# LBM-EPFL/MaD

Hardware: NVIDIA B200
Metric: voxels/sec scale-space+detect+describe(+match) (higher is better)
Workload: dtype f32 grids, f64 line accumulation, u8 x u8 -> s32 matching

## Files before the change

### include/mad_b200.h

```cpp
#ifndef MAD_B200_H
#define MAD_B200_H

#include <stddef.h>
#include <stdint.h>

#ifdef __cplusplus
extern "C" {
#endif

#define MAD_OK 0
#define MAD_ERR_ARG (-1)
#define MAD_ERR_CUDA (-2)
#define MAD_ERR_CAPACITY (-3)
#define MAD_ERR_NODEVICE (-4)

#define MAD_MAX_ORI 36
#define MAD_DSC_LEN 1024
#define MAD_DSC_REFUSED (1 << 30)

typedef struct MadKeypoint {
    int32_t vox[3];
    int32_t oct;
    float off[3];
    float val;
    int32_t peak[3];
    int32_t accepted;
} MadKeypoint;

typedef struct MadOriented {
    int32_t kp;
    int16_t main_bin;
    int16_t sec_bin;
} MadOriented;

typedef struct MadZoneTable {
    int32_t n_zones;
    int32_t n_belts;
    const double* bounds;
    const int32_t* belt_first;
    const double* belt_phi;
    const void* fast;
} MadZoneTable;

#define MAD_ZONE_FAST_BYTES 2048
int mad_zone_fast_build(const MadZoneTable* zones_host, void* fast_out, void* stream);

const char* mad_last_error_string(void);
int mad_version(void);
int mad_device_info(int* sm_count, int* cc_major, int* cc_minor);

int mad_publish_small(const void* src_dev, void* dst_host_mapped, int bytes, void* stream);

int mad_copy_to_host(const void* src_dev, void* dst_host_mapped, long long bytes, int n_ctas, void* stream);

long long mad_launch_count(void);
int mad_profile_enable(int on);
int mad_profile_count(void);
int mad_profile_get(int i, const char** name, float* ms);
int mad_profile_reset(void);

int mad_grid_max(const float* grid, long long n, float* out_max_ord, void* stream);
float mad_grid_max_decode(unsigned int ord);
int mad_threshold_normalise(float* grid, long long n, float isovalue, float vmax, int divide, void* stream);
int mad_grid_bbox(const float* grid, int nx, int ny, int nz, int* bbox6, void* stream);
int mad_crop_pad3d(const float* in, int nx, int ny, int nz, int x0, int y0, int z0, int cx, int cy, int cz,
                   int pad, float* out, void* stream);

int mad_pad3d(const float* in, int nx, int ny, int nz, int pad, float* out, void* stream);

size_t mad_upsample_workspace_bytes(int bx, int by, int bz);
int mad_upsample_presmooth(const float* base, int bx, int by, int bz,
                           const double* gauss_w_host, int radius,
                           float* up, void* workspace, size_t workspace_bytes, void* stream);

size_t mad_log_gauss_workspace_bytes(int nx, int ny, int nz);
int mad_log_gauss(const float* grid, int nx, int ny, int nz,
                  const double* w0_host, const double* w2_host, int radius, float scale,
                  float* log_out, float* gauss_out, void* workspace, size_t workspace_bytes,
                  int exact_f64, void* stream);

int mad_gradient(const float* gauss, int nx, int ny, int nz, float* grad4, void* stream);
size_t mad_gradient_tiles(int nx, int ny, int nz);
int mad_gradient_mark(const MadKeypoint* kp, int n_kp, const int* dims_oct_host, int reach_oct0, int reach_oct1,
                      uint8_t* flags_oct0, uint8_t* flags_oct1, void* stream);
int mad_gradient_masked(const float* gauss, int nx, int ny, int nz, float* grad4, uint8_t* flags, void* stream);

int mad_detect(const float* log_grid, int nx, int ny, int nz, int oct, int border,
               float threshold, MadKeypoint* cand, int cap, int* count, void* stream);

size_t mad_sort_keypoints_workspace_bytes(int n);
int mad_sort_keypoints(const MadKeypoint* cand, int n, const int* dims_oct_host,
                       MadKeypoint* out, int* out_count,
                       void* workspace, size_t workspace_bytes, void* stream);

int mad_orient(const float* grad4_oct0, const float* grad4_oct1, const int* dims_oct_host,
               const MadKeypoint* kp, int n_kp, int r, const MadZoneTable* zones112_host,
               const double* r1_table, int lim_main, int lim_sec,
               int32_t* n_ori, int32_t* slots, void* stream);

size_t mad_compact_oriented_workspace_bytes(int n_kp);
int mad_compact_oriented(const int32_t* n_ori, const int32_t* slots, int n_kp,
                         MadOriented* oriented, int cap, int* out_count,
                         void* workspace, size_t workspace_bytes, void* stream);

int mad_describe(const float* grad4_oct0, const float* grad4_oct1, const int* dims_oct_host,
                 const MadKeypoint* kp, const MadOriented* oriented, int n_oriented, int r,
                 const MadZoneTable* zones16_host, const double* rf_table, const double* rf_inv_table,
                 int rf_zones, int16_t* dsc, void* stream);

typedef struct MadDscSet {
    const int16_t* dsc;
    const void* half;
    const int32_t* norm2;
    const uint8_t* u8;
    const float* rnorm;
    int32_t rows;
    int32_t rows_padded;
    int32_t max_entry;
    int32_t max_norm2;
} MadDscSet;

int mad_dsc_prepare(const int16_t* dsc, int rows, int rows_padded, int32_t* norm2, float* rnorm,
                    uint8_t* u8, int32_t* max_entry, int32_t* max_norm2, void* stream);
int mad_dsc_norms(const int16_t* dsc, int rows, int32_t* norm2, void* stream);
int mad_dsc_to_half(const int16_t* dsc, int rows, int rows_padded, void* half_out, void* stream);

int mad_match_segments(int M, int N, int impl);
int mad_match_count(const MadDscSet* hi, const MadDscSet* lo, double cc, int n_seg, int32_t* seg_count, int impl,
                    void* stream);
int mad_match_fill(const MadDscSet* hi, const MadDscSet* lo, double cc, int n_seg, const int64_t* seg_offset,
                   int32_t* pair_hi, int32_t* pair_lo, double* pair_score, int impl, void* stream);
size_t mad_exclusive_scan_workspace_bytes(int n);
int mad_exclusive_scan_i32_to_i64(const int32_t* in, int n, int64_t* out, int64_t* total,
                                  void* workspace, size_t workspace_bytes, void* stream);

int mad_match_pairs(const MadDscSet* hi, const MadDscSet* lo, double cc, uint64_t* cand_key, int32_t* cand_dot,
                    uint64_t cap, uint64_t* count, void* stream);
size_t mad_match_pairs_finish_workspace_bytes(long long n);
int mad_match_pairs_finish(const uint64_t* cand_key, const int32_t* cand_dot, long long n, int hi_rows, int lo_rows,
                           const int32_t* hi_n2, const int32_t* lo_n2, int32_t* pair_hi, int32_t* pair_lo,
                           double* pair_score, void* workspace, size_t workspace_bytes, void* stream);
int mad_match_pairs_finish_dot(const uint64_t* cand_key, const int32_t* cand_dot, long long n, int hi_rows, int lo_rows,
                               int32_t* pair_hi, int32_t* pair_lo, int32_t* pair_dot, void* workspace, size_t workspace_bytes,
                               void* stream);

size_t mad_match_topk_workspace_bytes(int M, int N, int k, int impl);
int mad_match_topk(const MadDscSet* hi, const MadDscSet* lo, int k, int lo_index_base,
                   int32_t* topk_idx, double* topk_score, void* workspace, size_t workspace_bytes,
                   int impl, void* stream);
#define MAD_TOPK_INCOMPLETE (-2)
int mad_topk_merge(const int32_t* idx_in, const double* score_in, int G, int M, int k,
                   int32_t* idx_out, double* score_out, void* stream);

int mad_mark_used(const int32_t* idx, long long n, uint8_t* used, void* stream);
int mad_repeatability(const int32_t* pair_hi, const int32_t* pair_lo, const double* pair_score, long long n_pairs,
                      const double* hi_subv, const double* lo_subv, const int32_t* hi_meta, const int32_t* lo_meta,
                      const double* rf_table, const double* rf_inv_table, int rf_zones,
                      const double* hi_cloud, int n_hi_cloud, const double* lo_sorted, const int32_t* cell_start,
                      const uint32_t* near_bits, const double* grid_org_host, const int* grid_dims_host,
                      double dist, double* results, void* stream);
int mad_repeat_counts(const int32_t* pair_hi, const int32_t* pair_lo, long long p0, long long p1,
                      const double* hi_subv, const double* lo_subv, const int32_t* hi_meta, const int32_t* lo_meta,
                      const double* rf_table, const double* rf_inv_table, int rf_zones,
                      const double* hi_cloud, int n_hi_cloud, const double* lo_sorted, const int32_t* cell_start,
                      const uint32_t* near_bits, const double* grid_org_host, const int* grid_dims_host,
                      double dist, int32_t* counts, void* stream);
int mad_repeat_rows(const int32_t* pair_hi, const int32_t* pair_lo, const double* pair_score, long long n_pairs,
                    const double* hi_subv, const double* lo_subv, const int32_t* hi_meta, const int32_t* lo_meta,
                    const double* rf_table, const double* rf_inv_table, int rf_zones, const int32_t* counts,
                    int n_hi_cloud, double* results, void* stream);

size_t mad_anchor_cloud_workspace_bytes(int n_rows);
int mad_anchor_cloud(const double* subv, const uint8_t* used, int n_rows, double cell, double* cloud, double* grid_org,
                     long long* info, void* workspace, size_t workspace_bytes, void* stream);
size_t mad_cloud_grid_workspace_bytes(int n);
int mad_cloud_grid(const double* cloud, int n, const double* grid_org, const long long* grid_dims_host, double cell,
                   double* sorted, int32_t* cell_start, uint32_t* near_bits, void* workspace, size_t workspace_bytes,
                   void* stream);

int mad_density_splat(const double* xyz, const double* mass, int n_atoms, const double* min_host, double voxelsp,
                      int margin, int px, int py, int pz, double* grid, void* stream);
int mad_normalise_f64(double* grid, long long n, void* scratch8, void* stream);
int mad_conv_full_f64(const double* in, long long outer, int n, long long inner, const double* w_dev, int radius,
                      void* out, int out_is_f32, void* stream);

size_t mad_box_scores_workspace_bytes(int ex, int ey, int ez);
int mad_box_scores(const float* g1, int nx1, int ny1, int nz1, const float* g2, int nx2, int ny2, int nz2,
                   const int* box_host, float isovalue, double* out8, void* workspace, size_t workspace_bytes,
                   void* stream);
int mad_grid_count_gt(const float* grid, long long n, float thr, unsigned long long* out, void* stream);
int mad_mask_with(float* g1, int nx1, int ny1, int nz1, const float* g2, int nx2, int ny2, int nz2,
                  const int* shift_host, const int* lo_host, const int* hi_host, void* stream);
int mad_refine_rigid(const float* grad4, int nx, int ny, int nz, const double* px, const double* py, const double* pz,
                     double voxsp, const double* init, const double* center, const double* max_dist, int n_problems,
                     int n_atoms, int n_steps, double max_step, double min_step, double* coords_out, double* meta_out,
                     void* stream);

#ifdef __cplusplus
}
#endif
#endif
```

### mad_b200/_lib.py

```python
import ctypes as C
import os

import numpy as np

HERE = os.path.dirname(os.path.abspath(__file__))
LIB_PATH = os.path.join(HERE, "libmad_b200.so")


class MadError(RuntimeError):
    pass


if not os.path.exists(LIB_PATH):
    raise ImportError(
        "mad_b200: %s is missing -- build the CUDA library first (python -m mad_b200.build). "
        "There is no CPU fallback." % LIB_PATH)

lib = C.CDLL(LIB_PATH)

KEYPOINT_DTYPE = np.dtype([("vox", "<i4", 3), ("oct", "<i4"), ("off", "<f4", 3), ("val", "<f4"),
                           ("peak", "<i4", 3), ("accepted", "<i4")])
ORIENTED_DTYPE = np.dtype([("kp", "<i4"), ("main", "<i2"), ("sec", "<i2")])
assert KEYPOINT_DTYPE.itemsize == 48 and ORIENTED_DTYPE.itemsize == 8
MAX_ORI = 36
DSC_LEN = 1024
DSC_REFUSED = 1 << 30
TOPK_INCOMPLETE = -2
TOPK_MAX = 32
ZONE_FAST_BYTES = 2048


class MadZoneTable(C.Structure):
    _fields_ = [("n_zones", C.c_int32), ("n_belts", C.c_int32), ("bounds", C.c_void_p),
                ("belt_first", C.c_void_p), ("belt_phi", C.c_void_p), ("fast", C.c_void_p)]


class MadDscSet(C.Structure):
    _fields_ = [("dsc", C.c_void_p), ("half", C.c_void_p), ("norm2", C.c_void_p), ("u8", C.c_void_p),
                ("rnorm", C.c_void_p), ("rows", C.c_int32), ("rows_padded", C.c_int32), ("max_entry", C.c_int32),
                ("max_norm2", C.c_int32)]


_P = C.c_void_p
_I = C.c_int
_SZ = C.c_size_t

SIGNATURES = {
    "mad_last_error_string": (C.c_char_p, []),
    "mad_version": (_I, []),
    "mad_device_info": (_I, [C.POINTER(_I), C.POINTER(_I), C.POINTER(_I)]),
    "mad_launch_count": (C.c_longlong, []),
    "mad_profile_enable": (_I, [_I]),
    "mad_profile_count": (_I, []),
    "mad_profile_get": (_I, [_I, C.POINTER(C.c_char_p), C.POINTER(C.c_float)]),
    "mad_profile_reset": (_I, []),
    "mad_publish_small": (_I, [_P, _P, _I, _P]),
    "mad_copy_to_host": (_I, [_P, _P, C.c_longlong, _I, _P]),
    "mad_zone_fast_build": (_I, [C.POINTER(MadZoneTable), _P, _P]),
    "mad_grid_max": (_I, [_P, C.c_longlong, _P, _P]),
    "mad_grid_max_decode": (C.c_float, [C.c_uint]),
    "mad_threshold_normalise": (_I, [_P, C.c_longlong, C.c_float, C.c_float, _I, _P]),
    "mad_grid_bbox": (_I, [_P, _I, _I, _I, _P, _P]),
    "mad_crop_pad3d": (_I, [_P, _I, _I, _I, _I, _I, _I, _I, _I, _I, _I, _P, _P]),
    "mad_pad3d": (_I, [_P, _I, _I, _I, _I, _P, _P]),
    "mad_upsample_workspace_bytes": (_SZ, [_I, _I, _I]),
    "mad_upsample_presmooth": (_I, [_P, _I, _I, _I, _P, _I, _P, _P, _SZ, _P]),
    "mad_log_gauss_workspace_bytes": (_SZ, [_I, _I, _I]),
    "mad_log_gauss": (_I, [_P, _I, _I, _I, _P, _P, _I, C.c_float, _P, _P, _P, _SZ, _I, _P]),
    "mad_gradient": (_I, [_P, _I, _I, _I, _P, _P]),
    "mad_gradient_tiles": (_SZ, [_I, _I, _I]),
    "mad_gradient_mark": (_I, [_P, _I, _P, _I, _I, _P, _P, _P]),
    "mad_gradient_masked": (_I, [_P, _I, _I, _I, _P, _P, _P]),
    "mad_detect": (_I, [_P, _I, _I, _I, _I, _I, C.c_float, _P, _I, _P, _P]),
    "mad_sort_keypoints_workspace_bytes": (_SZ, [_I]),
    "mad_sort_keypoints": (_I, [_P, _I, _P, _P, _P, _P, _SZ, _P]),
    "mad_orient": (_I, [_P, _P, _P, _P, _I, _I, C.POINTER(MadZoneTable), _P, _I, _I, _P, _P, _P]),
    "mad_compact_oriented_workspace_bytes": (_SZ, [_I]),
    "mad_compact_oriented": (_I, [_P, _P, _I, _P, _I, _P, _P, _SZ, _P]),
    "mad_describe": (_I, [_P, _P, _P, _P, _P, _I, _I, C.POINTER(MadZoneTable), _P, _P, _I, _P, _P]),
    "mad_dsc_prepare": (_I, [_P, _I, _I, _P, _P, _P, _P, _P, _P]),
    "mad_match_pairs": (_I, [C.POINTER(MadDscSet), C.POINTER(MadDscSet), C.c_double, _P, _P, C.c_uint64, _P, _P]),
    "mad_match_pairs_finish_workspace_bytes": (_SZ, [C.c_longlong]),
    "mad_match_pairs_finish": (_I, [_P, _P, C.c_longlong, _I, _I, _P, _P, _P, _P, _P, _P, _SZ, _P]),
    "mad_match_pairs_finish_dot": (_I, [_P, _P, C.c_longlong, _I, _I, _P, _P, _P, _P, _SZ, _P]),
    "mad_dsc_norms": (_I, [_P, _I, _P, _P]),
    "mad_dsc_to_half": (_I, [_P, _I, _I, _P, _P]),
    "mad_match_segments": (_I, [_I, _I, _I]),
    "mad_match_count": (_I, [C.POINTER(MadDscSet), C.POINTER(MadDscSet), C.c_double, _I, _P, _I, _P]),
    "mad_match_fill": (_I, [C.POINTER(MadDscSet), C.POINTER(MadDscSet), C.c_double, _I, _P, _P, _P, _P, _I, _P]),
    "mad_exclusive_scan_workspace_bytes": (_SZ, [_I]),
    "mad_exclusive_scan_i32_to_i64": (_I, [_P, _I, _P, _P, _P, _SZ, _P]),
    "mad_match_topk_workspace_bytes": (_SZ, [_I, _I, _I, _I]),
    "mad_match_topk": (_I, [C.POINTER(MadDscSet), C.POINTER(MadDscSet), _I, _I, _P, _P, _P, _SZ, _I, _P]),
    "mad_topk_merge": (_I, [_P, _P, _I, _I, _I, _P, _P, _P]),
    "mad_density_splat": (_I, [_P, _P, _I, _P, C.c_double, _I, _I, _I, _I, _P, _P]),
    "mad_normalise_f64": (_I, [_P, C.c_longlong, _P, _P]),
    "mad_conv_full_f64": (_I, [_P, C.c_longlong, _I, C.c_longlong, _P, _I, _P, _I, _P]),
    "mad_mark_used": (_I, [_P, C.c_longlong, _P, _P]),
    "mad_repeatability": (_I, [_P, _P, _P, C.c_longlong, _P, _P, _P, _P, _P, _P, _I, _P, _I, _P, _P, _P, _P, _P,
                               C.c_double, _P, _P]),
    "mad_repeat_counts": (_I, [_P, _P, C.c_longlong, C.c_longlong, _P, _P, _P, _P, _P, _P, _I, _P, _I, _P, _P, _P, _P, _P,
                               C.c_double, _P, _P]),
    "mad_repeat_rows": (_I, [_P, _P, _P, C.c_longlong, _P, _P, _P, _P, _P, _P, _I, _P, _I, _P, _P]),
    "mad_anchor_cloud_workspace_bytes": (_SZ, [_I]),
    "mad_anchor_cloud": (_I, [_P, _P, _I, C.c_double, _P, _P, _P, _P, _SZ, _P]),
    "mad_cloud_grid_workspace_bytes": (_SZ, [_I]),
    "mad_cloud_grid": (_I, [_P, _I, _P, _P, C.c_double, _P, _P, _P, _P, _SZ, _P]),
    "mad_box_scores_workspace_bytes": (_SZ, [_I, _I, _I]),
    "mad_box_scores": (_I, [_P, _I, _I, _I, _P, _I, _I, _I, _P, C.c_float, _P, _P, _SZ, _P]),
    "mad_grid_count_gt": (_I, [_P, C.c_longlong, C.c_float, _P, _P]),
    "mad_mask_with": (_I, [_P, _I, _I, _I, _P, _I, _I, _I, _P, _P, _P, _P]),
    "mad_refine_rigid": (_I, [_P, _I, _I, _I, _P, _P, _P, C.c_double, _P, _P, _P, _I, _I, _I, C.c_double, C.c_double,
                              _P, _P, _P]),
}

for _name, (_res, _args) in SIGNATURES.items():
    _f = getattr(lib, _name)
    _f.restype = _res
    _f.argtypes = _args


def last_error():
    s = lib.mad_last_error_string()
    return s.decode() if s else ""


def check(rc, what):
    if rc != 0:
        raise MadError("%s failed with status %d: %s" % (what, rc, last_error()))


def call(name, *args):
    check(getattr(lib, name)(*args), name)
```

### mad_b200/csrc/match_common.cuh

```cuda
#pragma once
#include <math.h>
#include "common.cuh"

#define MAD_TOPK_MAX 32

__host__ __device__ __forceinline__ double mad_score(int dot, double n2a, double n2b) {
    const double p = n2a * n2b;
    return p > 0.0 ? (double)dot / sqrt(p) : 0.0;
}

__host__ __device__ __forceinline__ void mad_topk_insert(double* bs, int* bi, int k, double s, int id) {
    const double ls = bs[k - 1];
    const int li = bi[k - 1];
    if (!(s > ls || (s == ls && (li < 0 || id < li)))) return;
    int q = k - 1;
    while (q > 0) {
        const double ps = bs[q - 1];
        const int pi = bi[q - 1];
        if (s > ps || (s == ps && (pi < 0 || id < pi))) { bs[q] = ps; bi[q] = pi; --q; }
        else break;
    }
    bs[q] = s;
    bi[q] = id;
}

__host__ __device__ __forceinline__ bool mad_topk_before(double s, int id, double ps, int pi) {
    return s > ps || (s == ps && (pi < 0 || id < pi));
}

__device__ __forceinline__ void mad_top8_insert(double (&bs)[8], int (&bi)[8], double s, int id) {
    bool c[8];
#pragma unroll
    for (int q = 0; q < 8; ++q) c[q] = mad_topk_before(s, id, bs[q], bi[q]);
#pragma unroll
    for (int q = 7; q >= 1; --q) {
        bs[q] = c[q - 1] ? bs[q - 1] : (c[q] ? s : bs[q]);
        bi[q] = c[q - 1] ? bi[q - 1] : (c[q] ? id : bi[q]);
    }
    bs[0] = c[0] ? s : bs[0];
    bi[0] = c[0] ? id : bi[0];
}

static __device__ __noinline__ bool mad_score_before_nl(int d, int n, int id, int pd, int pn, int pi, double n2a) {
    return mad_topk_before(mad_score(d, n2a, (double)n), id, mad_score(pd, n2a, (double)pn), pi);
}
__device__ __forceinline__ bool mad_score32_before(float s, int d, int n, int id, float ps, int pd, int pn, int pi, double n2a) {
    if (pi < 0) return true;
    const float tol = 4e-6f * fmaxf(s, ps);
    if (s > ps + tol) return true;
    if (s < ps - tol) return false;
    return mad_score_before_nl(d, n, id, pd, pn, pi, n2a);
}

__device__ __forceinline__ void mad_top8f_insert(float (&ts)[8], int (&td)[8], int (&tn)[8], int (&bi)[8], bool active, float s,
                                                 int d, int n, int id, double n2a) {
    bool c[8];
    bool amb = false;
#pragma unroll
    for (int q = 0; q < 8; ++q) {
        const float ps = ts[q];
        const bool empty = bi[q] < 0;
        const float tol = 4e-6f * fmaxf(s, ps);
        const bool gt = s > ps + tol, lt = s < ps - tol;
        c[q] = active && (empty || gt);
        amb |= active && !empty && !gt && !lt;
    }
    if (__any_sync(0xFFFFFFFFu, amb)) {
#pragma unroll
        for (int q = 0; q < 8; ++q) c[q] = active && mad_score32_before(s, d, n, id, ts[q], td[q], tn[q], bi[q], n2a);
    }
#pragma unroll
    for (int q = 7; q >= 1; --q) {
        ts[q] = c[q - 1] ? ts[q - 1] : (c[q] ? s : ts[q]);
        td[q] = c[q - 1] ? td[q - 1] : (c[q] ? d : td[q]);
        tn[q] = c[q - 1] ? tn[q - 1] : (c[q] ? n : tn[q]);
        bi[q] = c[q - 1] ? bi[q - 1] : (c[q] ? id : bi[q]);
    }
    ts[0] = c[0] ? s : ts[0];
    td[0] = c[0] ? d : td[0];
    tn[0] = c[0] ? n : tn[0];
    bi[0] = c[0] ? id : bi[0];
}

__device__ __forceinline__ void mad_st_release_cta(volatile int* p, int v) {
    asm volatile("st.release.cta.shared::cta.s32 [%0], %1;" ::"r"((uint32_t)__cvta_generic_to_shared((const void*)p)), "r"(v) : "memory");
}
__device__ __forceinline__ int mad_ld_acquire_cta(volatile int* p) {
    int v;
    asm volatile("ld.acquire.cta.shared::cta.s32 %0, [%1];" : "=r"(v) : "r"((uint32_t)__cvta_generic_to_shared((const void*)p)) : "memory");
    return v;
}

__device__ __forceinline__ uint32_t mad_select32(const uint32_t (&v)[32], int j) {
    uint32_t a[16];
#pragma unroll
    for (int i = 0; i < 16; ++i) a[i] = (j & 1) ? v[2 * i + 1] : v[2 * i];
    uint32_t b[8];
#pragma unroll
    for (int i = 0; i < 8; ++i) b[i] = (j & 2) ? a[2 * i + 1] : a[2 * i];
    uint32_t c[4];
#pragma unroll
    for (int i = 0; i < 4; ++i) c[i] = (j & 4) ? b[2 * i + 1] : b[2 * i];
    const uint32_t d0 = (j & 8) ? c[1] : c[0], d1 = (j & 8) ? c[3] : c[2];
    return (j & 16) ? d1 : d0;
}

#define MAD_MATCH_SEG_TILE 256

int mad_check_descriptor_sets(const MadDscSet* hi, const MadDscSet* lo, const char* who);

int mad_match_simt(const int16_t* hi, int M, const int16_t* lo, int N, const int32_t* hi_n2, const int32_t* lo_n2,
                   double cc, int mode, int S, int32_t* seg_count, const int64_t* seg_offset, int32_t* pair_hi,
                   int32_t* pair_lo, double* pair_score, int k, int lo_index_base, int32_t* topk_idx,
                   double* topk_score, cudaStream_t st);

int mad_match_tc_segments(int M, int N);
int mad_match_tc(const void* hi_half, int M, int M_pad, const void* lo_half, int N, int N_pad,
                 const int32_t* hi_n2, const int32_t* lo_n2, double cc, int mode, int S, int32_t* seg_count,
                 const int64_t* seg_offset, int32_t* pair_hi, int32_t* pair_lo, double* pair_score, int k,
                 int lo_index_base, int32_t* topk_idx, double* topk_score, cudaStream_t st);
int mad_topk_merge_launch(const int32_t* idx_in, const double* score_in, int G, int M, int k, int32_t* idx_out,
                          double* score_out, cudaStream_t st);

int mad_match_u8_segments(int M, int N);
int mad_match_u8_segments_topk(int M, int N);
int mad_match_u8_pairs(const void* hi_u8, int M, int M_pad, const void* lo_u8, int N, int N_pad, const int32_t* hi_n2,
                       const int32_t* lo_n2, const float* lo_rnorm, double cc, unsigned long long* cand_key,
                       int32_t* cand_dot, unsigned long long cap, unsigned long long* count, cudaStream_t st);
int mad_match_u8_topk(const void* hi_u8, int M, int M_pad, const void* lo_u8, int N, int N_pad, const int32_t* hi_n2,
                      const int32_t* lo_n2, const float* lo_rnorm, int S, int k, int lo_index_base, int32_t* topk_idx,
                      double* topk_score, cudaStream_t st);
```

### mad_b200/csrc/match_prep.cu

```cuda
#include <cub/cub.cuh>

#include "common.cuh"
#include "match_common.cuh"

namespace {

__global__ void __launch_bounds__(256)
dsc_prepare_kernel(const int16_t* __restrict__ dsc, int rows, int rows_padded, int32_t* __restrict__ norm2,
                   float* __restrict__ rnorm, uint8_t* __restrict__ u8, int32_t* __restrict__ max_entry,
                   int32_t* __restrict__ max_norm2) {
    const int row = (int)((blockIdx.x * (long long)blockDim.x + threadIdx.x) >> 5);
    const int lane = threadIdx.x & 31;
    if (row >= rows_padded) return;
    long long acc = 0;
    int mx = 0;
    uint32_t packed[8];
    if (row < rows) {
        const uint4* src = reinterpret_cast<const uint4*>(dsc + (long long)row * MAD_DSC_LEN + lane * 32);
#pragma unroll
        for (int q = 0; q < 4; ++q) {
            const uint4 v = __ldg(src + q);
            const uint32_t w[4] = {v.x, v.y, v.z, v.w};
#pragma unroll
            for (int h = 0; h < 4; ++h) {
                const int e0 = (int)(int16_t)(w[h] & 0xFFFFu), e1 = (int)(int16_t)(w[h] >> 16);
                acc += (long long)e0 * e0 + (long long)e1 * e1;
                mx = max(mx, max(e0, e1));
                if (e0 < 0 || e1 < 0) mx = MAD_DSC_REFUSED;
                const uint32_t b0 = (uint32_t)min(max(e0, 0), 255), b1 = (uint32_t)min(max(e1, 0), 255);
                const int slot = q * 8 + h * 2;
                if ((slot & 3) == 0) packed[slot >> 2] = b0 | (b1 << 8);
                else packed[slot >> 2] |= (b0 << 16) | (b1 << 24);
            }
        }
    } else {
#pragma unroll
        for (int q = 0; q < 8; ++q) packed[q] = 0;
    }
    if (u8) {
        uint4* dst = reinterpret_cast<uint4*>(u8 + (long long)row * MAD_DSC_LEN + lane * 32);
        dst[0] = make_uint4(packed[0], packed[1], packed[2], packed[3]);
        dst[1] = make_uint4(packed[4], packed[5], packed[6], packed[7]);
    }
#pragma unroll
    for (int o = 16; o > 0; o >>= 1) {
        acc += __shfl_xor_sync(0xFFFFFFFFu, acc, o);
        mx = max(mx, __shfl_xor_sync(0xFFFFFFFFu, mx, o));
    }
    if (lane == 0) {
        if (acc > 0x7FFFFFFFLL) mx = MAD_DSC_REFUSED;
        if (row < rows) norm2[row] = (int32_t)acc;
        rnorm[row] = acc > 0 ? (float)(1.0 / sqrt((double)acc)) : 0.f;
        if (mx > 0) atomicMax(max_entry, mx);
        if (max_norm2 && acc > 0) atomicMax(max_norm2, (int32_t)min(acc, 0x7FFFFFFFLL));
    }
}

__global__ void pairs_finish_kernel(const unsigned long long* __restrict__ key, const int32_t* __restrict__ dot,
                                    long long n, unsigned long long lo_rows, const int32_t* __restrict__ hi_n2,
                                    const int32_t* __restrict__ lo_n2,
                                    int32_t* __restrict__ pair_hi, int32_t* __restrict__ pair_lo,
                                    double* __restrict__ score) {
    const long long i = blockIdx.x * (long long)blockDim.x + threadIdx.x;
    if (i >= n) return;
    const unsigned long long k = key[i];
    const int row = (int)(k / lo_rows), col = (int)(k % lo_rows);
    pair_hi[i] = row;
    pair_lo[i] = col;
    score[i] = mad_score(dot[i], (double)__ldg(hi_n2 + row), (double)__ldg(lo_n2 + col));
}

__global__ void pairs_finish_dot_kernel(const unsigned long long* __restrict__ key, const int32_t* __restrict__ dot, long long n,
                                        unsigned long long lo_rows, int32_t* __restrict__ pair_hi, int32_t* __restrict__ pair_lo,
                                        int32_t* __restrict__ pair_dot) {
    const long long i = blockIdx.x * (long long)blockDim.x + threadIdx.x;
    if (i >= n) return;
    const unsigned long long k = key[i];
    pair_hi[i] = (int)(k / lo_rows);
    pair_lo[i] = (int)(k % lo_rows);
    pair_dot[i] = dot[i];
}

__global__ void zero_u64_kernel(unsigned long long* p) { *p = 0ull; }

struct FinishLayout {
    size_t key_off, dot_off, cub_off, cub_bytes, total;
};

FinishLayout finish_layout(long long n) {
    FinishLayout L;
    const size_t nn = (size_t)(n > 0 ? n : 1);
    L.key_off = 0;
    L.dot_off = mad_align_up(nn * sizeof(unsigned long long), 256);
    L.cub_off = L.dot_off + mad_align_up(nn * sizeof(int32_t), 256);
    size_t b = 0;
    cub::DeviceRadixSort::SortPairs(nullptr, b, (const unsigned long long*)nullptr, (unsigned long long*)nullptr,
                                    (const int32_t*)nullptr, (int32_t*)nullptr, (int)nn, 0, 64);
    L.cub_bytes = mad_align_up(b, 256);
    L.total = L.cub_off + L.cub_bytes;
    return L;
}

}

extern "C" int mad_dsc_prepare(const int16_t* dsc, int rows, int rows_padded, int32_t* norm2, float* rnorm,
                               uint8_t* u8, int32_t* max_entry, int32_t* max_norm2, void* stream) {
    MAD_CHECK_ARG(rows >= 0 && rows_padded >= rows);
    if (rows_padded == 0) return MAD_OK;
    MAD_CHECK_ARG((rows == 0 || dsc) && norm2 && rnorm && max_entry);
    MAD_CHECK_ARG((reinterpret_cast<uintptr_t>(dsc) & 15) == 0 && (reinterpret_cast<uintptr_t>(u8) & 15) == 0);
    MAD_PROF("dsc_prepare_kernel", stream);
    dsc_prepare_kernel<<<(unsigned)mad_ceil_div((long long)rows_padded * 32, 256), 256, 0, (cudaStream_t)stream>>>(
        dsc, rows, rows_padded, norm2, rnorm, u8, max_entry, max_norm2);
    MAD_LAUNCH_OK();
    return MAD_OK;
}

extern "C" int mad_match_pairs(const MadDscSet* hi, const MadDscSet* lo, double cc, uint64_t* cand_key, int32_t* cand_dot,
                               uint64_t cap, uint64_t* count, void* stream) {
    MAD_CHECK_ARG(hi && lo && count && hi->rows >= 0 && lo->rows >= 0);
    cudaStream_t st = (cudaStream_t)stream;
    {
        MAD_PROF("zero_u64_kernel", st);
        zero_u64_kernel<<<1, 1, 0, st>>>(reinterpret_cast<unsigned long long*>(count));
        MAD_LAUNCH_OK();
    }
    if (hi->rows == 0 || lo->rows == 0) return MAD_OK;
    MAD_CHECK_ARG(hi->u8 && lo->u8 && hi->norm2 && lo->norm2 && lo->rnorm && cand_key && cand_dot);
    MAD_CHECK_ARG(hi->rows_padded >= hi->rows && hi->rows_padded % 128 == 0);
    MAD_CHECK_ARG(lo->rows_padded >= lo->rows && lo->rows_padded % 128 == 0);
    int rc = mad_check_descriptor_sets(hi, lo, "mad_match_pairs");
    if (rc != MAD_OK) return rc;
    if (hi->max_entry > 255 || lo->max_entry > 255) {
        mad_set_error("mad_match_pairs: descriptor entries up to %d do not fit the uint8 tensor-core operand "
                      "(use mad_match_count/mad_match_fill with impl = 2 or 1)",
                      hi->max_entry > lo->max_entry ? hi->max_entry : lo->max_entry);
        return MAD_ERR_ARG;
    }
    return mad_match_u8_pairs(hi->u8, hi->rows, hi->rows_padded, lo->u8, lo->rows, lo->rows_padded, hi->norm2, lo->norm2,
                              lo->rnorm, cc, reinterpret_cast<unsigned long long*>(cand_key), cand_dot,
                              (unsigned long long)cap, reinterpret_cast<unsigned long long*>(count), st);
}

extern "C" size_t mad_match_pairs_finish_workspace_bytes(long long n) { return finish_layout(n).total; }

static int pairs_finish_impl(const uint64_t* cand_key, const int32_t* cand_dot, long long n, int hi_rows, int lo_rows,
                             const int32_t* hi_n2, const int32_t* lo_n2, int32_t* pair_hi, int32_t* pair_lo, double* pair_score,
                             int32_t* pair_dot, void* workspace, size_t workspace_bytes, void* stream);

extern "C" int mad_match_pairs_finish(const uint64_t* cand_key, const int32_t* cand_dot, long long n, int hi_rows,
                                      int lo_rows, const int32_t* hi_n2, const int32_t* lo_n2, int32_t* pair_hi, int32_t* pair_lo,
                                      double* pair_score, void* workspace, size_t workspace_bytes, void* stream) {
    MAD_CHECK_ARG(n >= 0 && n < (1LL << 31));
    if (n == 0) return MAD_OK;
    MAD_CHECK_ARG(hi_n2 && lo_n2 && pair_score);
    return pairs_finish_impl(cand_key, cand_dot, n, hi_rows, lo_rows, hi_n2, lo_n2, pair_hi, pair_lo, pair_score, nullptr, workspace,
                             workspace_bytes, stream);
}

extern "C" int mad_match_pairs_finish_dot(const uint64_t* cand_key, const int32_t* cand_dot, long long n, int hi_rows, int lo_rows,
                                          int32_t* pair_hi, int32_t* pair_lo, int32_t* pair_dot, void* workspace,
                                          size_t workspace_bytes, void* stream) {
    MAD_CHECK_ARG(n >= 0 && n < (1LL << 31));
    if (n == 0) return MAD_OK;
    MAD_CHECK_ARG(pair_dot);
    return pairs_finish_impl(cand_key, cand_dot, n, hi_rows, lo_rows, nullptr, nullptr, pair_hi, pair_lo, nullptr, pair_dot, workspace,
                             workspace_bytes, stream);
}

static int pairs_finish_impl(const uint64_t* cand_key, const int32_t* cand_dot, long long n, int hi_rows, int lo_rows,
                             const int32_t* hi_n2, const int32_t* lo_n2, int32_t* pair_hi, int32_t* pair_lo, double* pair_score,
                             int32_t* pair_dot, void* workspace, size_t workspace_bytes, void* stream) {
    MAD_CHECK_ARG(cand_key && cand_dot && pair_hi && pair_lo && workspace && hi_rows > 0 && lo_rows > 0);
    const FinishLayout L = finish_layout(n);
    MAD_CHECK_ARG(workspace_bytes >= L.total);
    cudaStream_t st = (cudaStream_t)stream;
    char* ws = reinterpret_cast<char*>(workspace);
    unsigned long long* key_sorted = reinterpret_cast<unsigned long long*>(ws + L.key_off);
    int32_t* dot_sorted = reinterpret_cast<int32_t*>(ws + L.dot_off);
    int key_bits = 1;
    while (key_bits < 64 && (1ULL << key_bits) < (unsigned long long)hi_rows * (unsigned long long)lo_rows) ++key_bits;
    size_t b = L.cub_bytes;
    {
        MAD_PROF("cub_radix_sort_pairs", st);
        MAD_CUDA(cub::DeviceRadixSort::SortPairs(ws + L.cub_off, b, reinterpret_cast<const unsigned long long*>(cand_key),
                                                 key_sorted, cand_dot, dot_sorted, (int)n, 0, key_bits, st));
    }
    MAD_PROF("pairs_finish_kernel", st);
    if (pair_dot)
        pairs_finish_dot_kernel<<<(unsigned)mad_ceil_div(n, 256), 256, 0, st>>>(key_sorted, dot_sorted, n, (unsigned long long)lo_rows, pair_hi,
                                                                               pair_lo, pair_dot);
    else
        pairs_finish_kernel<<<(unsigned)mad_ceil_div(n, 256), 256, 0, st>>>(key_sorted, dot_sorted, n, (unsigned long long)lo_rows, hi_n2, lo_n2,
                                                                           pair_hi, pair_lo, pair_score);
    MAD_LAUNCH_OK();
    return MAD_OK;
}
```

### mad_b200/csrc/match_u8.cu

```cuda
#include <cuda.h>
#include <stdlib.h>

#include <type_traits>

#include "common.cuh"
#include "match_common.cuh"

namespace {

constexpr int BM = 128;
constexpr int BN = 128;
constexpr int BKB = 128;
constexpr int UKB = 32;
constexpr int KBLOCKS = MAD_DSC_LEN / BKB;
constexpr int STAGES = 5;
constexpr int STAGES2 = 10;
constexpr int ACCS = 4;
constexpr uint32_t KB_BYTES = BM * BKB;
constexpr uint32_t A_BYTES = KBLOCKS * KB_BYTES;
constexpr int EPI_WARPS = 8;
constexpr int THREADS = 128 + 32 * EPI_WARPS + 64;
constexpr uint32_t TMEM_COLS = 512;
constexpr unsigned long long MAD_MATCH_TIMEOUT_COUNT = 1ull << 62;
constexpr int STG = 96;
constexpr size_t STG_BYTES = (size_t)EPI_WARPS * STG * (sizeof(unsigned long long) + sizeof(int));
constexpr size_t RB_BYTES = (size_t)2 * 2 * 256 * sizeof(float);
constexpr size_t THR_BYTES = 512;
constexpr int TOP_SLOTS = 2;
constexpr int TOP_LOCAL_TILES = 4;
constexpr unsigned long long TOP_INVALID = ~0ull;
static_assert((size_t)EPI_WARPS * 2 * 32 * TOP_SLOTS * sizeof(unsigned long long) <= STG_BYTES, "TOP8 slots fit the staging area");
constexpr size_t SMEM_BYTES = 1024 + A_BYTES + (size_t)STAGES * KB_BYTES + STG_BYTES + RB_BYTES + 512 + THR_BYTES;
static_assert(SMEM_BYTES <= 232448, "shared memory budget of one sm_100 CTA");

__device__ __forceinline__ uint32_t smem_u32(const void* p) { return (uint32_t)__cvta_generic_to_shared(p); }
__device__ __forceinline__ void mbar_init(uint32_t bar, uint32_t count) {
    asm volatile("mbarrier.init.shared::cta.b64 [%0], %1;" ::"r"(bar), "r"(count) : "memory");
}
__device__ __forceinline__ void mbar_expect_tx(uint32_t bar, uint32_t bytes) {
    asm volatile("mbarrier.arrive.expect_tx.shared::cta.b64 _, [%0], %1;" ::"r"(bar), "r"(bytes) : "memory");
}
__device__ __forceinline__ void mbar_arrive(uint32_t bar) {
    asm volatile("mbarrier.arrive.shared::cta.b64 _, [%0];" ::"r"(bar) : "memory");
}
__device__ __forceinline__ void mbar_wait(uint32_t bar, uint32_t parity) {
    uint32_t done;
    do {
        asm volatile(
            "{\n\t.reg .pred p;\n\t"
            "mbarrier.try_wait.parity.shared::cta.b64 p, [%1], %2;\n\t"
            "selp.u32 %0, 1, 0, p;\n\t}"
            : "=r"(done)
            : "r"(bar), "r"(parity)
            : "memory");
    } while (!done);
}
__device__ __forceinline__ void tma_load_2d(uint32_t dst, const CUtensorMap* map, uint32_t bar, int c0, int c1) {
    asm volatile(
        "cp.async.bulk.tensor.2d.shared::cluster.global.mbarrier::complete_tx::bytes [%0], [%1, {%3, %4}], [%2];"
        ::"r"(dst), "l"(reinterpret_cast<uint64_t>(map)), "r"(bar), "r"(c0), "r"(c1)
        : "memory");
}
constexpr uint32_t kPeerBitMask = 0xFEFFFFFFu;
__device__ __forceinline__ uint32_t cluster_ctarank() {
    uint32_t r;
    asm volatile("mov.u32 %0, %%cluster_ctarank;" : "=r"(r));
    return r;
}
__device__ __forceinline__ void cluster_sync_all() {
    asm volatile("barrier.cluster.arrive.release.aligned;" ::: "memory");
    asm volatile("barrier.cluster.wait.acquire.aligned;" ::: "memory");
}
__device__ __forceinline__ void tma_load_2d_2sm(uint32_t dst, const CUtensorMap* map, uint32_t bar, int c0, int c1) {
    asm volatile(
        "cp.async.bulk.tensor.2d.cta_group::2.shared::cluster.global.mbarrier::complete_tx::bytes [%0], [%1, {%3, %4}], [%2];"
        ::"r"(dst), "l"(reinterpret_cast<uint64_t>(map)), "r"(bar & kPeerBitMask), "r"(c0), "r"(c1)
        : "memory");
}
__device__ __forceinline__ void mbar_arrive_leader(uint32_t bar) {
    asm volatile("mbarrier.arrive.shared::cluster.b64 _, [%0];" ::"r"(bar & kPeerBitMask) : "memory");
}
__device__ __forceinline__ void umma_commit_pair(uint32_t bar) {
    asm volatile("tcgen05.commit.cta_group::2.mbarrier::arrive::one.shared::cluster.multicast::cluster.b64 [%0], %1;"
                 ::"r"(bar), "h"((uint16_t)3) : "memory");
}
__device__ __forceinline__ void umma_i8_pair(uint32_t d_tmem, uint64_t a_desc, uint64_t b_desc, uint32_t idesc, uint32_t accumulate) {
    asm volatile(
        "{\n\t.reg .pred p;\n\t"
        "setp.ne.b32 p, %4, 0;\n\t"
        "tcgen05.mma.cta_group::2.kind::i8 [%0], %1, %2, %3, p;\n\t}"
        ::"r"(d_tmem), "l"(a_desc), "l"(b_desc), "r"(idesc), "r"(accumulate)
        : "memory");
}
__device__ __forceinline__ void umma_commit(uint32_t bar) {
    asm volatile("tcgen05.commit.cta_group::1.mbarrier::arrive::one.shared::cluster.b64 [%0];" ::"r"(bar) : "memory");
}
__device__ __forceinline__ void umma_i8(uint32_t d_tmem, uint64_t a_desc, uint64_t b_desc, uint32_t idesc, uint32_t accumulate) {
    asm volatile(
        "{\n\t.reg .pred p;\n\t"
        "setp.ne.b32 p, %4, 0;\n\t"
        "tcgen05.mma.cta_group::1.kind::i8 [%0], %1, %2, %3, p;\n\t}"
        ::"r"(d_tmem), "l"(a_desc), "l"(b_desc), "r"(idesc), "r"(accumulate)
        : "memory");
}
__device__ __forceinline__ void tmem_ld32(uint32_t taddr, uint32_t (&v)[32]) {
    asm volatile(
        "tcgen05.ld.sync.aligned.32x32b.x32.b32 "
        "{%0, %1, %2, %3, %4, %5, %6, %7, %8, %9, %10, %11, %12, %13, %14, %15, "
        "%16, %17, %18, %19, %20, %21, %22, %23, %24, %25, %26, %27, %28, %29, %30, %31}, [%32];"
        : "=r"(v[0]), "=r"(v[1]), "=r"(v[2]), "=r"(v[3]), "=r"(v[4]), "=r"(v[5]), "=r"(v[6]), "=r"(v[7]),
          "=r"(v[8]), "=r"(v[9]), "=r"(v[10]), "=r"(v[11]), "=r"(v[12]), "=r"(v[13]), "=r"(v[14]), "=r"(v[15]),
          "=r"(v[16]), "=r"(v[17]), "=r"(v[18]), "=r"(v[19]), "=r"(v[20]), "=r"(v[21]), "=r"(v[22]), "=r"(v[23]),
          "=r"(v[24]), "=r"(v[25]), "=r"(v[26]), "=r"(v[27]), "=r"(v[28]), "=r"(v[29]), "=r"(v[30]), "=r"(v[31])
        : "r"(taddr)
        : "memory");
}
__device__ __forceinline__ uint32_t tmem_ld1(uint32_t taddr) {
    uint32_t x;
    asm volatile("tcgen05.ld.sync.aligned.32x32b.x1.b32 {%0}, [%1];" : "=r"(x) : "r"(taddr) : "memory");
    return x;
}
__device__ __forceinline__ void tmem_ld_wait() { asm volatile("tcgen05.wait::ld.sync.aligned;" ::: "memory"); }
__device__ __forceinline__ void tc_fence_before() { asm volatile("tcgen05.fence::before_thread_sync;" ::: "memory"); }
__device__ __forceinline__ void tc_fence_after() { asm volatile("tcgen05.fence::after_thread_sync;" ::: "memory"); }

__device__ __forceinline__ uint64_t umma_smem_desc(uint32_t saddr) {
    uint64_t d = 0;
    d |= (uint64_t)((saddr & 0x3FFFFu) >> 4);
    d |= (uint64_t)1 << 16;
    d |= (uint64_t)(1024u >> 4) << 32;
    d |= (uint64_t)1 << 46;
    d |= (uint64_t)2 << 61;
    return d;
}
constexpr uint32_t kIdesc = (2u << 4) | ((uint32_t)(BN >> 3) << 17) | ((uint32_t)(BM >> 4) << 24);
constexpr uint32_t kIdescPair = (2u << 4) | ((uint32_t)((2 * BN) >> 3) << 17) | ((uint32_t)((2 * BM) >> 4) << 24);

struct U8Args {
    int M, N, S;
    int tiles_per_seg;
    const int32_t* hi_n2;
    const int32_t* lo_n2;
    const float* lo_rnorm;
    double cc;
    unsigned long long* cand_key;
    int32_t* cand_dot;
    unsigned long long cap;
    unsigned long long* count;
    int k, lo_index_base;
    int local_tiles;
    int dbg;
    int32_t* topk_idx;
    double* topk_score;
};

__device__ unsigned long long g_top_dbg[8];

enum { MODE_PAIRS = 0, MODE_TOPK = 1, MODE_TOP8 = 2 };

template <int MODE, int NCTA>
__global__ void __launch_bounds__(THREADS, 1)
match_u8_kernel(const __grid_constant__ CUtensorMap map_hi, const __grid_constant__ CUtensorMap map_lo, U8Args a) {
    constexpr int TN = (NCTA == 2) ? 2 * BN : BN;
    constexpr int NACC = (int)TMEM_COLS / TN;
    constexpr int NSTAGE = STAGES;
    constexpr uint32_t SB = KB_BYTES;
    extern __shared__ uint8_t smem_raw[];
    const uint32_t raw = smem_u32(smem_raw);
    const uint32_t base = (raw + 1023u) & ~1023u;
    uint8_t* gen = smem_raw + (base - raw);
    const uint32_t b_ring = base + A_BYTES;
    constexpr uint32_t STG_OFF = A_BYTES + STAGES * KB_BYTES;
    unsigned long long* stg_key = reinterpret_cast<unsigned long long*>(gen + STG_OFF);
    int* stg_dot = reinterpret_cast<int*>(gen + STG_OFF + EPI_WARPS * STG * sizeof(unsigned long long));
    float* s_rb = reinterpret_cast<float*>(gen + STG_OFF + (uint32_t)STG_BYTES);
    constexpr uint32_t BAR_OFF = STG_OFF + (uint32_t)(STG_BYTES + RB_BYTES);
    const uint32_t bars = base + BAR_OFF;
    auto full_bar = [&](int s) { return bars + 8u * s; };
    auto empty_bar = [&](int s) { return bars + 8u * (NSTAGE + s); };
    auto tfull_bar = [&](int q) { return bars + 8u * (2 * NSTAGE + q); };
    auto tempty_bar = [&](int q) { return bars + 8u * (2 * NSTAGE + ACCS + q); };
    const uint32_t a_bar = bars + 8u * (2 * NSTAGE + 2 * ACCS);
    uint32_t* tmem_slot = reinterpret_cast<uint32_t*>(gen + BAR_OFF + 8 * (2 * NSTAGE + 2 * ACCS + 1));
    volatile int* s_half = reinterpret_cast<volatile int*>(gen + BAR_OFF + 8 * (2 * NSTAGE + 2 * ACCS + 2));
    volatile int* s_done = s_half + 2 * EPI_WARPS;
    static_assert(8 * (2 * STAGES + 2 * ACCS + 2) + 3 * EPI_WARPS * sizeof(int) <= 512, "misc shared region");
    volatile unsigned long long* top_slots = reinterpret_cast<volatile unsigned long long*>(gen + STG_OFF);
    volatile float* s_thr8 = reinterpret_cast<volatile float*>(gen + BAR_OFF + 512);

    const int warp = threadIdx.x >> 5, lane = threadIdx.x & 31;
    const uint32_t rank = (NCTA == 2) ? cluster_ctarank() : 0u;
    const int m0 = blockIdx.x * BM;
    const int seg = blockIdx.y;
    const int n_tiles_total = (a.N + TN - 1) / TN;
    const int t_begin = seg * a.tiles_per_seg;
    const int t_end = min(n_tiles_total, t_begin + a.tiles_per_seg);

    if (threadIdx.x == 0) {
        for (int s = 0; s < NSTAGE; ++s) { mbar_init(full_bar(s), 1); mbar_init(empty_bar(s), 1); }
        for (int q = 0; q < NACC; ++q) { mbar_init(tfull_bar(q), 1); mbar_init(tempty_bar(q), NCTA == 2 ? 16 : 4); }
        mbar_init(a_bar, 1);
        asm volatile("fence.mbarrier_init.release.cluster;" ::: "memory");
    }
    if (threadIdx.x < 3 * EPI_WARPS) s_half[threadIdx.x] = 0;
    volatile float* s_thr = reinterpret_cast<volatile float*>(gen + STG_OFF);
    if (MODE == MODE_TOPK && threadIdx.x < 2 * BM) s_thr[threadIdx.x] = -1.f;
    if (MODE == MODE_TOP8) {
        for (int i = threadIdx.x; i < EPI_WARPS * 2 * 32 * TOP_SLOTS; i += THREADS) top_slots[i] = TOP_INVALID;
        if (threadIdx.x < BM) s_thr8[threadIdx.x] = -1.f;
    }
    if (NCTA == 2) cluster_sync_all();
    if (warp == 2) {
        if (NCTA == 2) {
            asm volatile("tcgen05.alloc.cta_group::2.sync.aligned.shared::cta.b32 [%0], %1;" ::"r"(smem_u32(tmem_slot)), "n"(TMEM_COLS) : "memory");
            asm volatile("tcgen05.relinquish_alloc_permit.cta_group::2.sync.aligned;" ::: "memory");
        } else {
            asm volatile("tcgen05.alloc.cta_group::1.sync.aligned.shared::cta.b32 [%0], %1;" ::"r"(smem_u32(tmem_slot)), "n"(TMEM_COLS) : "memory");
            asm volatile("tcgen05.relinquish_alloc_permit.cta_group::1.sync.aligned;" ::: "memory");
        }
    }
    tc_fence_before();
    __syncthreads();
    tc_fence_after();
    const uint32_t tmem_base = *tmem_slot;

    if (warp == 0) {
        if (lane == 0) {
            if (NCTA == 2) {
                if (rank == 0) mbar_expect_tx(a_bar, 2 * A_BYTES);
                for (int kb = 0; kb < KBLOCKS; ++kb) tma_load_2d_2sm(base + kb * KB_BYTES, &map_hi, a_bar, kb * BKB, m0);
            } else {
                mbar_expect_tx(a_bar, A_BYTES);
                for (int kb = 0; kb < KBLOCKS; ++kb) tma_load_2d(base + kb * KB_BYTES, &map_hi, a_bar, kb * BKB, m0);
            }
            int stage = 0;
            uint32_t phase = 0;
            for (int t = t_begin; t < t_end; ++t) {
                for (int kb = 0; kb < KBLOCKS; ++kb) {
                    mbar_wait(empty_bar(stage), phase ^ 1u);
                    if (NCTA == 2) {
                        if (rank == 0) mbar_expect_tx(full_bar(stage), 2 * KB_BYTES);
                        tma_load_2d_2sm(b_ring + stage * SB, &map_lo, full_bar(stage), kb * BKB, t * TN + (int)rank * BN);
                    } else {
                        mbar_expect_tx(full_bar(stage), KB_BYTES);
                        tma_load_2d(b_ring + stage * SB, &map_lo, full_bar(stage), kb * BKB, t * BN);
                    }
                    if (++stage == NSTAGE) { stage = 0; phase ^= 1u; }
                }
            }
        }
    } else if (warp == 1) {
        if (lane == 0 && rank == 0) {
            mbar_wait(a_bar, 0);
            tc_fence_after();
            int stage = 0;
            uint32_t phase = 0;
            int it = 0;
            for (int t = t_begin; t < t_end; ++t, ++it) {
                const int acc = it % NACC;
                const uint32_t acc_phase = (uint32_t)(it / NACC) & 1u;
                mbar_wait(tempty_bar(acc), acc_phase ^ 1u);
                tc_fence_after();
                const uint32_t d_tmem = tmem_base + (uint32_t)(acc * TN);
                for (int kb = 0; kb < KBLOCKS; ++kb) {
                    mbar_wait(full_bar(stage), phase);
                    tc_fence_after();
                    const uint64_t da = umma_smem_desc(base + kb * KB_BYTES);
                    const uint64_t db = umma_smem_desc(b_ring + stage * SB);
#pragma unroll
                    for (int kk = 0; kk < BKB / UKB; ++kk) {
                        if (NCTA == 2) umma_i8_pair(d_tmem, da + (uint64_t)(2 * kk), db + (uint64_t)(2 * kk), kIdescPair, (kb | kk) ? 1u : 0u);
                        else umma_i8(d_tmem, da + (uint64_t)(2 * kk), db + (uint64_t)(2 * kk), kIdesc, (kb | kk) ? 1u : 0u);
                    }
                    if (NCTA == 2) umma_commit_pair(empty_bar(stage)); else umma_commit(empty_bar(stage));
                    if (++stage == NSTAGE) { stage = 0; phase ^= 1u; }
                }
                if (NCTA == 2) umma_commit_pair(tfull_bar(acc)); else umma_commit(tfull_bar(acc));
            }
        }
    } else if (warp >= 2 && warp < 4 && MODE == MODE_PAIRS) {
        constexpr int HALF = STG / 2;
        const int e0 = (warp - 2) * 4;
        const double cc2 = a.cc * a.cc;
        int hi_n2_reg[4];
#pragma unroll
        for (int qq = 0; qq < 4; ++qq) hi_n2_reg[qq] = (m0 + qq * 32 + lane < a.M) ? __ldg(a.hi_n2 + m0 + qq * 32 + lane) : 0;
        for (long long spins = 0; spins < (1LL << 27); ++spins) {
            int done = 0;
            for (int e = e0; e < e0 + 4; ++e) done += mad_ld_acquire_cta(&s_done[e]);
            bool any = false;
            for (int e = e0; e < e0 + 4; ++e) {
                for (int h = 0; h < 2; ++h) {
                    const int n = mad_ld_acquire_cta(&s_half[2 * e + h]);
                    if (n <= 0) continue;
                    any = true;
                    const unsigned long long* hk = stg_key + e * STG + h * HALF;
                    const int* hd = stg_dot + e * STG + h * HALF;
                    unsigned long long ent[2];
                    int dot[2];
                    bool ok[2];
#pragma unroll
                    for (int k = 0; k < 2; ++k) {
                        const int i = lane + 32 * k;
                        ent[k] = (i < n) ? hk[i] : 0ull;
                        dot[k] = (i < n) ? hd[i] : 0;
                    }
                    __syncwarp();
                    if (lane == 0) mad_st_release_cta(&s_half[2 * e + h], 0);
                    int total = 0, pos[2];
                    const int qe = e & 3;
                    const int n2_q = qe == 0 ? hi_n2_reg[0] : (qe == 1 ? hi_n2_reg[1] : (qe == 2 ? hi_n2_reg[2] : hi_n2_reg[3]));
#pragma unroll
                    for (int k = 0; k < 2; ++k) {
                        ok[k] = false;
                        const unsigned low = (unsigned)ent[k];
                        const double n2r = (double)__shfl_sync(0xFFFFFFFFu, n2_q, (int)(low & 31u));
                        if (lane + 32 * k < n) {
                            const int row = m0 + qe * 32 + (int)(low & 31u);
                            const double n2c = (double)(unsigned)(ent[k] >> 32);
                            const double p = n2r * n2c, lhs = (double)dot[k] * (double)dot[k], rhs = cc2 * p;
                            if (p > 0.0 && a.cc > 0.0 && lhs > rhs * (1.0 + 1e-13)) ok[k] = true;
                            else if (p > 0.0 && a.cc > 0.0 && lhs < rhs * (1.0 - 1e-13)) ok[k] = false;
                            else ok[k] = mad_score(dot[k], n2r, n2c) > a.cc;
                            ent[k] = (unsigned long long)row * (unsigned long long)a.N + (unsigned long long)(low >> 5);
                        }
                        const unsigned m = __ballot_sync(0xFFFFFFFFu, ok[k]);
                        pos[k] = total + __popc(m & ((1u << lane) - 1u));
                        total += __popc(m);
                    }
                    if (total > 0) {
                        unsigned long long gb = 0;
                        if (lane == 0) gb = atomicAdd(a.count, (unsigned long long)total);
                        gb = __shfl_sync(0xFFFFFFFFu, gb, 0);
#pragma unroll
                        for (int k = 0; k < 2; ++k)
                            if (ok[k] && gb + pos[k] < a.cap) { a.cand_key[gb + pos[k]] = ent[k]; a.cand_dot[gb + pos[k]] = dot[k]; }
                    }
                }
            }
            if (!any) {
                if (done == 4) break;
                __nanosleep(200);
            }
            if (spins == (1LL << 27) - 1 && lane == 0) atomicExch(a.count, MAD_MATCH_TIMEOUT_COUNT);
        }
    } else if ((warp == 2 || warp == 3 || warp >= 4 + EPI_WARPS) && MODE == MODE_TOP8) {
        const int dq = warp < 4 ? warp - 2 : warp - (4 + EPI_WARPS) + 2;
        float ts[8];
        int td[8], tn[8], bi[8];
#pragma unroll
        for (int i = 0; i < 8; ++i) { ts[i] = 0.f; td[i] = 0; tn[i] = 1; bi[i] = -1; }
        const int row = m0 + 32 * dq + lane;
        const int n2a_i = row < a.M ? __ldg(a.hi_n2 + row) : 0;
        const float ra = n2a_i > 0 ? (float)(1.0 / sqrt((double)n2a_i)) : 0.f;
        bool timeout = false;
        for (long long spins = 0;; ++spins) {
            if (spins >= (1LL << 26)) { timeout = true; break; }
            const int done = mad_ld_acquire_cta(&s_done[dq]) + mad_ld_acquire_cta(&s_done[4 + dq]);
            bool any = false;
#pragma unroll 1
            for (int g = 0; g < 2; ++g) {
                const int e = g * 4 + dq;
#pragma unroll 1
                for (int h = 0; h < 2; ++h) {
                    const int tt = mad_ld_acquire_cta(&s_half[2 * e + h]);
                    if (tt <= 0) continue;
                    any = true;
                    const long long dc0 = (a.dbg & 32) ? clock64() : 0;
                    int n_ins = 0, n_stale = 0;
                    volatile unsigned long long* sl = top_slots + ((e * 2 + h) * 32 + lane) * TOP_SLOTS;
                    unsigned long long ent[TOP_SLOTS];
#pragma unroll
                    for (int u = 0; u < TOP_SLOTS; ++u) { ent[u] = sl[u]; sl[u] = TOP_INVALID; }
                    __syncwarp();
                    if (lane == 0) mad_st_release_cta(&s_half[2 * e + h], 0);
                    const int colbase = a.lo_index_base + (tt - 1) * TN;
                    bool changed = false;
#pragma unroll
                    for (int u = 0; u < TOP_SLOTS; ++u) {
                        const bool has = ent[u] != TOP_INVALID && !(a.dbg & 1);
                        if (!__any_sync(0xFFFFFFFFu, has)) continue;
                        const int dot = (int)(ent[u] >> 35), n2b = (int)((ent[u] >> 8) & 0x7FFFFFFull);
                        const int id = colbase + (int)(ent[u] & 0xFFull);
                        const bool nz = n2a_i > 0 && n2b > 0;
                        const float s32 = nz ? (float)dot * rsqrtf((float)n2b) * ra : 0.f;
                        const bool live = has && (bi[7] < 0 || s32 >= ts[7] * (1.f - 4e-6f));
                        if (!__any_sync(0xFFFFFFFFu, live)) { n_stale += has; continue; }
                        mad_top8f_insert(ts, td, tn, bi, live, s32, nz ? dot : 0, nz ? n2b : 1, id, (double)n2a_i);
                        changed |= live;
                        n_ins += live;
                        n_stale += has && !live;
                    }
                    if (a.dbg & 32) {
                        n_ins = __reduce_add_sync(0xFFFFFFFFu, n_ins);
                        n_stale = __reduce_add_sync(0xFFFFFFFFu, n_stale);
                        if (lane == 0) {
                            atomicAdd(&g_top_dbg[4], 1ull); atomicAdd(&g_top_dbg[5], (unsigned long long)(clock64() - dc0));
                            atomicAdd(&g_top_dbg[6], (unsigned long long)n_ins); atomicAdd(&g_top_dbg[7], (unsigned long long)n_stale);
                        }
                    }
                    if (changed && bi[7] >= 0) atomicMax(reinterpret_cast<int*>(const_cast<float*>(&s_thr8[dq * 32 + lane])), __float_as_int(fmaxf(ts[7] - 4e-6f, 0.f)));
                }
            }
            if (!any) {
                if (done == 2) break;
                __nanosleep(a.dbg & 16 ? 32 : (a.dbg & 64 ? 1000 : 300));
            }
        }
        if (row < a.M) {
            const long long o = ((long long)(seg * 3) * a.M + row) * a.k;
#pragma unroll
            for (int i = 0; i < 8; ++i)
                if (i < a.k) {
                    a.topk_idx[o + i] = timeout ? MAD_TOPK_INCOMPLETE : bi[i];
                    a.topk_score[o + i] = bi[i] < 0 ? -INFINITY : (td[i] == 0 ? 0.0 : mad_score(td[i], (double)n2a_i, (double)tn[i]));
                }
        }
    } else if (warp >= 4 && warp < 4 + EPI_WARPS) {
        const int q = warp & 3;
        const int ew = warp - 4;
        const int grp = ew >> 2;
        const int row = m0 + q * 32 + lane;
        const bool row_ok = row < a.M;
        const int n2a_i = row_ok ? a.hi_n2[row] : 0;
        const double n2a = (double)n2a_i;
        const float ra = n2a_i > 0 ? (float)(1.0 / sqrt(n2a)) : 0.f;
        const float thr_pairs = !row_ok ? INFINITY : (n2a_i > 0 ? ((float)a.cc - 4e-6f) / ra : (a.cc < 0.0 ? -INFINITY : INFINITY));
        unsigned long long* my_key = stg_key + ew * STG;
        int* my_dot = stg_dot + ew * STG;
        constexpr bool kTop = (MODE == MODE_TOPK || MODE == MODE_TOP8);
        constexpr int kList = (MODE == MODE_TOPK) ? MAD_TOPK_MAX : 1;
        double bs[kList];
        int bi[kList];
        float thr = -1.f;
        if (MODE == MODE_TOPK) {
#pragma unroll
            for (int i = 0; i < kList; ++i) { bs[i] = -INFINITY; bi[i] = -1; }
        }
        const int k_last = a.k - 1;
        int top_cnt = 0;
        float ls[8];
        int ld[8], ln[8], li[8];
        if (MODE == MODE_TOP8) {
#pragma unroll
            for (int i = 0; i < 8; ++i) { ls[i] = 0.f; ld[i] = 0; ln[i] = 1; li[i] = -1; }
        }
        auto flush_local = [&]() {
            if (li[7] >= 0) atomicMax(reinterpret_cast<int*>(const_cast<float*>(&s_thr8[q * 32 + lane])), __float_as_int(fmaxf(ls[7] - 4e-6f, 0.f)));
            if (row_ok) {
                const long long o = ((long long)(seg * 3 + 1 + grp) * a.M + row) * a.k;
#pragma unroll
                for (int i = 0; i < 8; ++i)
                    if (i < a.k) {
                        a.topk_idx[o + i] = li[i];
                        a.topk_score[o + i] = li[i] < 0 ? -INFINITY : (ld[i] == 0 ? 0.0 : mad_score(ld[i], n2a, (double)ln[i]));
                    }
            }
        };
        int stg_n = 0;
        constexpr int HALF = STG / 2;
        static_assert(HALF >= 32, "a half buffer must take one ballot round");
        int cur = 0;
        auto publish = [&](int n) {
            __syncwarp();
            if (n > 0) {
                if (lane == 0) {
                    mad_st_release_cta(&s_half[2 * ew + cur], n);
                    long long spins = 0;
                    while (mad_ld_acquire_cta(&s_half[2 * ew + (cur ^ 1)]) != 0 && ++spins < (1LL << 27)) __nanosleep(64);
                    if (spins >= (1LL << 27)) atomicExch(a.count, MAD_MATCH_TIMEOUT_COUNT);
                }
                cur ^= 1;
                __syncwarp();
            }
        };
        auto publish_top = [&](int t) {
            __syncwarp();
            if (lane == 0) {
                mad_st_release_cta(&s_half[2 * ew + cur], t + 1);
                long long spins = 0;
                const long long c0 = (a.dbg & 32) ? clock64() : 0;
                while (mad_ld_acquire_cta(&s_half[2 * ew + (cur ^ 1)]) != 0 && ++spins < (1LL << 26)) __nanosleep(32);
                if (a.dbg & 32) { atomicAdd(&g_top_dbg[1], (unsigned long long)(clock64() - c0)); atomicAdd(&g_top_dbg[2], 1ull); }
            }
            cur ^= 1;
            top_cnt = 0;
            __syncwarp();
        };
        constexpr bool kSplitCols = (NCTA == 2);
        constexpr int kStep = kSplitCols ? 1 : 2;
        const int c_lo = kSplitCols ? grp * BN : 0;
        float* my_rb = s_rb + grp * 2 * 256;
        const int gt = threadIdx.x - 128 - grp * 128;
        auto stage_rb = [&](int t, int buf) {
            if (gt < BN / 4) {
                const float4 r4 = __ldg(reinterpret_cast<const float4*>(a.lo_rnorm + (long long)t * TN + c_lo) + gt);
                reinterpret_cast<float4*>(my_rb + buf * 256)[gt] = r4;
                {
                    const int c = t * TN + c_lo + 4 * gt;
                    int4 n4;
                    n4.x = (c < a.N) ? __ldg(a.lo_n2 + c) : 0;
                    n4.y = (c + 1 < a.N) ? __ldg(a.lo_n2 + c + 1) : 0;
                    n4.z = (c + 2 < a.N) ? __ldg(a.lo_n2 + c + 2) : 0;
                    n4.w = (c + 3 < a.N) ? __ldg(a.lo_n2 + c + 3) : 0;
                    reinterpret_cast<int4*>(my_rb + buf * 256 + 128)[gt] = n4;
                }
            }
        };
        auto group_sync = [&]() { asm volatile("bar.sync %0, 128;" ::"r"(1 + grp) : "memory"); };
        const int t_first = t_begin + (kSplitCols ? 0 : grp);
        int it = kSplitCols ? 0 : grp;
        int par = 0;
        if (t_first < t_end) stage_rb(t_first, 0);
        auto tile_body = [&](auto local_tag, const int t, const int it, const int par) {
            const int acc = it % NACC;
            const uint32_t acc_phase = (uint32_t)(it / NACC) & 1u;
            const int n0 = t * TN;
            constexpr bool top_local = decltype(local_tag)::value;
            group_sync();
            if (t + kStep < t_end) stage_rb(t + kStep, par ^ 1);
            const float* rbt = my_rb + par * 256 - c_lo;
            mbar_wait(tfull_bar(acc), acc_phase);
            tc_fence_after();
            const uint32_t taddr = tmem_base + ((uint32_t)(q * 32) << 16) + (uint32_t)(acc * TN);
#pragma unroll 1
            for (int c0 = c_lo; c0 < c_lo + BN; c0 += 32) {
                uint32_t v[32];
                tmem_ld32(taddr + (uint32_t)c0, v);
                tmem_ld_wait();
                if (c0 == c_lo + BN - 32 && !(a.dbg & 4)) {
                    tc_fence_before();
                    __syncwarp();
                    if (lane == 0) {
                        if (NCTA == 2) mbar_arrive_leader(tempty_bar(acc)); else mbar_arrive(tempty_bar(acc));
                    }
                }
                float thr_eff = thr;
                if (MODE == MODE_TOPK && kSplitCols) thr_eff = fmaxf(thr, s_thr[(grp ^ 1) * BM + q * 32 + lane]);
                if (MODE == MODE_TOP8)
                    thr_eff = top_local ? (li[7] < 0 ? -1.f : ls[7] - 4e-6f) : s_thr8[q * 32 + lane];
                const float lim = kTop ? (row_ok && ra > 0.f ? thr_eff / ra : INFINITY) : thr_pairs;
                unsigned mask = 0;
#pragma unroll
                for (int j4 = 0; j4 < 8; ++j4) {
                    const float4 r4 = reinterpret_cast<const float4*>(rbt + c0)[j4];
                    const float rb[4] = {r4.x, r4.y, r4.z, r4.w};
#pragma unroll
                    for (int u = 0; u < 4; ++u) {
                        const float sc = (float)(int)v[4 * j4 + u] * rb[u];
                        const bool pass = kTop ? (sc >= lim) : (sc > lim);
                        mask |= (pass ? 1u : 0u) << (4 * j4 + u);
                    }
                }
                if (MODE == MODE_TOPK && row_ok && ra == 0.f) mask = (bi[k_last] < 0) ? 0xFFFFFFFFu : 0u;
                if (MODE == MODE_TOP8) {
                    if (row_ok && ra == 0.f) mask = (t == t_begin && c0 == 0) ? 0xFFu : 0u;
                    const int left = a.N - (n0 + c0);
                    if (left < 32) mask &= (left <= 0) ? 0u : ((1u << left) - 1u);
                    if (a.dbg & 2) mask = 0u;
                    if (top_local) {
                        for (;;) {
                            if (__ballot_sync(0xFFFFFFFFu, mask != 0u) == 0u) break;
                            const bool has = mask != 0u;
                            const int j = has ? __ffs(mask) - 1 : 0;
                            mask &= mask - 1;
                            const int dot = (int)mad_select32(v, j);
                            const int n2b = __float_as_int(rbt[c0 + j + 128]);
                            const bool nz = n2a_i > 0 && n2b > 0;
                            const float s32 = nz ? (float)dot * rbt[c0 + j] * ra : 0.f;
                            const bool live = has && (li[7] < 0 || s32 >= ls[7] * (1.f - 4e-6f));
                            if (__any_sync(0xFFFFFFFFu, live))
                                mad_top8f_insert(ls, ld, ln, li, live, s32, nz ? dot : 0, nz ? n2b : 1, a.lo_index_base + n0 + c0 + j, n2a);
                        }
                        continue;
                    }
                    const long long rc0 = (a.dbg & 32) ? clock64() : 0;
                    int n_rounds = 0;
                    for (;;) {
                        const unsigned b = __ballot_sync(0xFFFFFFFFu, mask != 0u);
                        if (b == 0u) break;
                        ++n_rounds;
                        if (__ballot_sync(0xFFFFFFFFu, mask != 0u && top_cnt == TOP_SLOTS) != 0u) publish_top(t);
                        if (mask) {
                            const int j = __ffs(mask) - 1;
                            mask &= mask - 1;
                            const unsigned long long dot = (unsigned long long)mad_select32(v, j);
                            const unsigned long long n2b = (unsigned long long)(unsigned)__float_as_int(rbt[c0 + j + 128]);
                            top_slots[((ew * 2 + cur) * 32 + lane) * TOP_SLOTS + top_cnt] = (dot << 35) | (n2b << 8) | (unsigned long long)(c0 + j);
                            ++top_cnt;
                        }
                    }
                    if ((a.dbg & 32) && lane == 0 && n_rounds) {
                        atomicAdd(&g_top_dbg[0], (unsigned long long)(clock64() - rc0));
                        atomicAdd(&g_top_dbg[3], (unsigned long long)n_rounds);
                    }
                } else if (kTop) {
                    while (mask) {
                        const int j = __ffs(mask) - 1;
                        mask &= mask - 1;
                        const int dot = (int)mad_select32(v, j);
                        const int col = n0 + c0 + j;
                        if (col < a.N) {
                            const int n2b = __float_as_int(rbt[c0 + j + 128]);
                            {
                                const double s = mad_score(dot, n2a, (double)n2b);
                                mad_topk_insert(bs, bi, a.k, s, a.lo_index_base + col);
                                thr = (bi[k_last] < 0) ? -1.f : (float)bs[k_last] - 4e-6f;
                                if (kSplitCols) s_thr[grp * BM + q * 32 + lane] = thr;
                            }
                        }
                    }
                } else {
                    const int left = a.N - (n0 + c0);
                    if (left < 32) mask &= (left <= 0) ? 0u : ((1u << left) - 1u);
                    const unsigned lt = (1u << lane) - 1u;
                    for (;;) {
                        const unsigned b = __ballot_sync(0xFFFFFFFFu, mask != 0u);
                        if (b == 0u) break;
                        const int nb = __popc(b);
                        if (stg_n + nb > HALF) { publish(stg_n); stg_n = 0; }
                        if (mask) {
                            const int j = __ffs(mask) - 1;
                            mask &= mask - 1;
                            const int p = cur * HALF + stg_n + __popc(b & lt);
                            my_key[p] = ((unsigned long long)(unsigned)__float_as_int(rbt[c0 + j + 128]) << 32) |
                                        (unsigned long long)(((unsigned)(n0 + c0 + j) << 5) | (unsigned)lane);
                            my_dot[p] = (int)mad_select32(v, j);
                        }
                        stg_n += nb;
                    }
                }
            }
            if (a.dbg & 4) {
                tc_fence_before();
                __syncwarp();
                if (lane == 0) { if (NCTA == 2) mbar_arrive_leader(tempty_bar(acc)); else mbar_arrive(tempty_bar(acc)); }
            }
            if (MODE == MODE_TOP8 && __ballot_sync(0xFFFFFFFFu, top_cnt > 0) != 0u) publish_top(t);
        };
        int t = t_first;
        if (MODE == MODE_TOP8) {
            for (int n = 0; n < a.local_tiles && t < t_end; ++n, t += kStep, it += kStep, par ^= 1) tile_body(std::true_type{}, t, it, par);
            flush_local();
        }
        for (; t < t_end; t += kStep, it += kStep, par ^= 1) tile_body(std::false_type{}, t, it, par);
        if (!kTop) {
            publish(stg_n);
            __syncwarp();
            if (lane == 0) mad_st_release_cta(&s_done[ew], 1);
        }
        if (MODE == MODE_TOP8) {
            __syncwarp();
            if (lane == 0) mad_st_release_cta(&s_done[ew], 1);
        }
        if (MODE == MODE_TOPK && row_ok) {
            const long long o = ((long long)(seg * 2 + grp) * a.M + row) * a.k;
            for (int i = 0; i < a.k; ++i) { a.topk_idx[o + i] = bi[i]; a.topk_score[o + i] = bs[i]; }
        }
    }
    tc_fence_before();
    __syncthreads();
    if (NCTA == 2) cluster_sync_all();
    if (warp == 2) {
        tc_fence_after();
        if (NCTA == 2) asm volatile("tcgen05.dealloc.cta_group::2.sync.aligned.b32 %0, %1;" ::"r"(tmem_base), "n"(TMEM_COLS) : "memory");
        else asm volatile("tcgen05.dealloc.cta_group::1.sync.aligned.b32 %0, %1;" ::"r"(tmem_base), "n"(TMEM_COLS) : "memory");
    }
}

typedef CUresult (*EncodeTiledFn)(CUtensorMap*, CUtensorMapDataType, cuuint32_t, void*, const cuuint64_t*, const cuuint64_t*,
                                  const cuuint32_t*, const cuuint32_t*, CUtensorMapInterleave, CUtensorMapSwizzle,
                                  CUtensorMapL2promotion, CUtensorMapFloatOOBfill);

EncodeTiledFn get_encode() {
    static EncodeTiledFn fn = nullptr;
    if (!fn) {
        void* p = nullptr;
        cudaDriverEntryPointQueryResult qres;
        if (cudaGetDriverEntryPoint("cuTensorMapEncodeTiled", &p, cudaEnableDefault, &qres) == cudaSuccess &&
            qres == cudaDriverEntryPointSuccess)
            fn = reinterpret_cast<EncodeTiledFn>(p);
    }
    return fn;
}

int make_map(CUtensorMap* map, const void* ptr, int rows_padded, int box_rows = BM) {
    EncodeTiledFn enc = get_encode();
    if (!enc) {
        mad_set_error("mad_match: cuTensorMapEncodeTiled is not available from the CUDA driver");
        return MAD_ERR_NODEVICE;
    }
    cuuint64_t dims[2] = {(cuuint64_t)MAD_DSC_LEN, (cuuint64_t)rows_padded};
    cuuint64_t strides[1] = {(cuuint64_t)MAD_DSC_LEN};
    cuuint32_t box[2] = {(cuuint32_t)BKB, (cuuint32_t)box_rows};
    cuuint32_t estr[2] = {1, 1};
    CUresult r = enc(map, CU_TENSOR_MAP_DATA_TYPE_UINT8, 2, const_cast<void*>(ptr), dims, strides, box, estr,
                     CU_TENSOR_MAP_INTERLEAVE_NONE, CU_TENSOR_MAP_SWIZZLE_128B, CU_TENSOR_MAP_L2_PROMOTION_L2_256B,
                     CU_TENSOR_MAP_FLOAT_OOB_FILL_NONE);
    if (r != CUDA_SUCCESS) {
        mad_set_error("mad_match: cuTensorMapEncodeTiled failed (%d)", (int)r);
        return MAD_ERR_CUDA;
    }
    return MAD_OK;
}

int check_device() {
    int dev = 0, major = 0;
    MAD_CUDA(cudaGetDevice(&dev));
    MAD_CUDA(cudaDeviceGetAttribute(&major, cudaDevAttrComputeCapabilityMajor, dev));
    if (major != 10) {
        mad_set_error("mad_match: the tcgen05 kernel needs an sm_100 device (found compute capability %d.x)", major);
        return MAD_ERR_NODEVICE;
    }
    return MAD_OK;
}

}

static int pick_ncta(int M, int N_pad);

static int u8_segments(int M, int N, double slack, int fixed_tiles) {
    if (M <= 0 || N <= 0) return 1;
    const int tn = pick_ncta(M, 256) == 2 ? 2 * BN : BN;
    const long long m_tiles = mad_ceil_div(M, BM);
    const long long n_tiles = mad_ceil_div(N, tn);
    const long long sms = mad_sm_count();
    long long best_s = 1, best_cost = -1;
    auto cost_of = [&](long long s) -> long long {
        const long long per = mad_ceil_div(n_tiles, s);
        const long long segs = mad_ceil_div(n_tiles, per);
        if (segs != s) return -1;
        return mad_ceil_div(m_tiles * s, sms) * (per + fixed_tiles);
    };
    for (long long s = 1; s <= n_tiles; ++s) {
        const long long cost = cost_of(s);
        if (cost < 0) continue;
        if (best_cost < 0 || cost < best_cost) { best_cost = cost; best_s = s; }
    }
    if (slack > 1.0)
        for (long long s = 1; s < best_s; ++s) {
            const long long cost = cost_of(s);
            if (cost >= 0 && (double)cost <= slack * (double)best_cost) return (int)s;
        }
    return (int)best_s;
}

int mad_match_u8_segments(int M, int N) { return u8_segments(M, N, 1.0, 1); }

int mad_match_u8_segments_topk(int M, int N) {
    static const int fixed = getenv("MAD_TOPK_FIXED_TILES") ? atoi(getenv("MAD_TOPK_FIXED_TILES")) : 53;
    return u8_segments(M, N, 1.0, fixed);
}

static int pick_ncta(int M, int N_pad) {
    static const bool one = getenv("MAD_MATCH_ONE_CTA") != nullptr;
    return (!one && M > BM && N_pad % 256 == 0) ? 2 : 1;
}

static int launch_common(const void* hi_u8, int M_pad, const void* lo_u8, int N_pad, int ncta, CUtensorMap* map_hi,
                         CUtensorMap* map_lo) {
    int rc = check_device();
    if (rc != MAD_OK) return rc;
    rc = make_map(map_hi, hi_u8, M_pad);
    if (rc != MAD_OK) return rc;
    (void)ncta;
    return make_map(map_lo, lo_u8, N_pad, BN);
}

template <int MODE>
static int launch_u8(int ncta, int M, int S, const CUtensorMap& map_hi, const CUtensorMap& map_lo, const U8Args& a,
                     cudaStream_t st) {
    if (ncta == 2) {
        auto kern = match_u8_kernel<MODE, 2>;
        MAD_CUDA(cudaFuncSetAttribute(kern, cudaFuncAttributeMaxDynamicSharedMemorySize, (int)SMEM_BYTES));
        cudaLaunchConfig_t cfg = {};
        cfg.gridDim = dim3(2u * (unsigned)mad_ceil_div(M, 2 * BM), (unsigned)S);
        cfg.blockDim = dim3(THREADS);
        cfg.dynamicSmemBytes = SMEM_BYTES;
        cfg.stream = st;
        cudaLaunchAttribute attr[1];
        attr[0].id = cudaLaunchAttributeClusterDimension;
        attr[0].val.clusterDim.x = 2;
        attr[0].val.clusterDim.y = 1;
        attr[0].val.clusterDim.z = 1;
        cfg.attrs = attr;
        cfg.numAttrs = 1;
        MAD_CUDA(cudaLaunchKernelEx(&cfg, kern, map_hi, map_lo, a));
    } else {
        auto kern = match_u8_kernel<MODE, 1>;
        MAD_CUDA(cudaFuncSetAttribute(kern, cudaFuncAttributeMaxDynamicSharedMemorySize, (int)SMEM_BYTES));
        dim3 grid((unsigned)mad_ceil_div(M, BM), (unsigned)S);
        kern<<<grid, THREADS, SMEM_BYTES, st>>>(map_hi, map_lo, a);
    }
    MAD_LAUNCH_OK();
    return MAD_OK;
}

int mad_match_u8_pairs(const void* hi_u8, int M, int M_pad, const void* lo_u8, int N, int N_pad, const int32_t* hi_n2,
                       const int32_t* lo_n2, const float* lo_rnorm, double cc, unsigned long long* cand_key,
                       int32_t* cand_dot, unsigned long long cap, unsigned long long* count, cudaStream_t st) {
    CUtensorMap map_hi, map_lo;
    const int ncta = pick_ncta(M, N_pad);
    int rc = launch_common(hi_u8, M_pad, lo_u8, N_pad, ncta, &map_hi, &map_lo);
    if (rc != MAD_OK) return rc;
    if (N_pad > (1 << 27)) { mad_set_error("mad_match_pairs: more than 2^27 lo rows"); return MAD_ERR_ARG; }
    U8Args a = {};
    a.M = M; a.N = N;
    a.S = mad_match_u8_segments(M, N);
    a.tiles_per_seg = (int)mad_ceil_div(mad_ceil_div(N, BN * ncta), a.S);
    a.hi_n2 = hi_n2; a.lo_n2 = lo_n2; a.lo_rnorm = lo_rnorm; a.cc = cc;
    a.cand_key = cand_key; a.cand_dot = cand_dot; a.cap = cap; a.count = count;
    a.dbg = getenv("MAD_TOPK_DBG") ? atoi(getenv("MAD_TOPK_DBG")) : 0;
    MAD_PROF("match_u8_pairs_kernel", st);
    return launch_u8<MODE_PAIRS>(ncta, M, a.S, map_hi, map_lo, a, st);
}

int mad_match_u8_topk(const void* hi_u8, int M, int M_pad, const void* lo_u8, int N, int N_pad, const int32_t* hi_n2,
                      const int32_t* lo_n2, const float* lo_rnorm, int S, int k, int lo_index_base, int32_t* topk_idx,
                      double* topk_score, cudaStream_t st) {
    CUtensorMap map_hi, map_lo;
    const int ncta = pick_ncta(M, N_pad);
    int rc = launch_common(hi_u8, M_pad, lo_u8, N_pad, ncta, &map_hi, &map_lo);
    if (rc != MAD_OK) return rc;
    U8Args a = {};
    a.M = M; a.N = N; a.S = S;
    a.tiles_per_seg = (int)mad_ceil_div(mad_ceil_div(N, BN * ncta), S);
    a.hi_n2 = hi_n2; a.lo_n2 = lo_n2; a.lo_rnorm = lo_rnorm; a.cc = 0.0;
    a.k = k; a.lo_index_base = lo_index_base; a.topk_idx = topk_idx; a.topk_score = topk_score;
    a.local_tiles = getenv("MAD_TOPK_LOCAL") ? atoi(getenv("MAD_TOPK_LOCAL")) : TOP_LOCAL_TILES;
    a.dbg = getenv("MAD_TOPK_DBG") ? atoi(getenv("MAD_TOPK_DBG")) : 0;
    if (a.dbg & 32) {
        unsigned long long z[8] = {0};
        cudaMemcpyToSymbolAsync(g_top_dbg, z, sizeof(z), 0, cudaMemcpyHostToDevice, st);
    }
    {
        MAD_PROF("match_u8_topk_kernel", st);
        rc = k <= 8 ? launch_u8<MODE_TOP8>(ncta, M, S, map_hi, map_lo, a, st) : launch_u8<MODE_TOPK>(ncta, M, S, map_hi, map_lo, a, st);
    }
    if (rc == MAD_OK && (a.dbg & 32)) {
        unsigned long long z[8];
        cudaStreamSynchronize(st);
        cudaMemcpyFromSymbol(z, g_top_dbg, sizeof(z));
        const double ctas = (double)(ncta == 2 ? 2 * mad_ceil_div(M, 2 * BM) : mad_ceil_div(M, BM)) * S;
        fprintf(stderr, "[top8 dbg] per CTA: round cycles %.0f (per epilogue warp %.0f), publish-wait cycles %.0f, publishes %.0f, rounds %.0f, "
                        "drain passes %.0f, drain busy cycles %.0f (per drain warp %.0f), inserted %.0f, stale %.0f\n",
                z[0] / ctas, z[0] / ctas / 8, z[1] / ctas, z[2] / ctas, z[3] / ctas, z[4] / ctas, z[5] / ctas, z[5] / ctas / 4, z[6] / ctas, z[7] / ctas);
    }
    return rc;
}
```

### mad_b200/pipeline.py

```python
import ctypes as C
import math
import os

import numpy as np
import torch

from . import _lib
from . import tables
from ._lib import call, KEYPOINT_DTYPE, ORIENTED_DTYPE, MAX_ORI, DSC_LEN

def launch_count():
    return int(_lib.lib.mad_launch_count())


def profile_enable(on=True):
    call("mad_profile_reset")
    call("mad_profile_enable", 1 if on else 0)


def profile_records():
    out = []
    name = C.c_char_p()
    ms = C.c_float()
    for i in range(_lib.lib.mad_profile_count()):
        call("mad_profile_get", i, C.byref(name), C.byref(ms))
        out.append((name.value.decode(), float(ms.value)))
    call("mad_profile_reset")
    return out


def _require_cuda():
    if not torch.cuda.is_available():
        raise _lib.MadError("mad_b200 needs a CUDA device (sm_100a); there is no CPU fallback")


def _stream():
    return C.c_void_p(torch.cuda.current_stream().cuda_stream)


def _ptr(t):
    return C.c_void_p(t.data_ptr()) if t is not None else C.c_void_p(0)


class _Readback(object):
    _slots = {}

    @classmethod
    def read(cls, *tensors):
        dev = tensors[0].device
        key = (dev.index, torch.cuda.current_stream().cuda_stream)
        slot = cls._slots.get(key)
        if slot is None:
            slot = cls._slots[key] = torch.zeros(512, dtype=torch.int64).pin_memory()
        st = _stream()
        off, views = 0, []
        for t in tensors:
            t = t.contiguous().view(-1)
            nbytes = t.numel() * t.element_size()
            assert nbytes % 4 == 0 and off + nbytes <= slot.numel() * 8
            call("mad_publish_small", _ptr(t), C.c_void_p(slot.data_ptr() + off), nbytes, st)
            views.append((off, t.dtype, t.numel()))
            off += (nbytes + 7) // 8 * 8
        torch.cuda.current_stream().synchronize()
        raw = slot.numpy()
        out = []
        for o, dt, n in views:
            a = raw.view(np.uint8)[o:o + n * (8 if dt == torch.int64 else 4)].view(np.int64 if dt == torch.int64 else np.int32)
            out.extend(int(v) for v in a)
        return out


def _dptr(a):
    return a.ctypes.data_as(C.c_void_p)


class _DeviceTables(object):

    def __init__(self, device, ori_zones=112, dsc_zones=16):
        self.device = device
        self.keep = []
        self.z_ori = self._zone_struct(tables.zone_tables(ori_zones))
        self.z_dsc = self._zone_struct(tables.zone_tables(dsc_zones))
        ot = tables.orientation_tables(ori_zones)
        self.ori_zones = ori_zones
        self.r1 = torch.from_numpy(np.ascontiguousarray(ot.r1.reshape(-1, 9))).to(device)
        self.rf = torch.from_numpy(np.ascontiguousarray(ot.rf.reshape(-1, 9))).to(device)
        self.rf_inv = torch.from_numpy(np.ascontiguousarray(ot.rf_inv.reshape(-1, 9))).to(device)

    def _zone_struct(self, zt):
        b = torch.from_numpy(np.ascontiguousarray(zt.bounds)).to(self.device)
        f = torch.from_numpy(np.ascontiguousarray(zt.belt_first)).to(self.device)
        p = torch.from_numpy(np.ascontiguousarray(zt.belt_phi)).to(self.device)
        self.keep += [b, f, p]
        s = _lib.MadZoneTable()
        s.n_zones, s.n_belts = zt.size, zt.n_belts
        s.bounds, s.belt_first, s.belt_phi = b.data_ptr(), f.data_ptr(), p.data_ptr()
        s.fast = None
        fast = torch.zeros(_lib.ZONE_FAST_BYTES, dtype=torch.uint8, device=self.device)
        with torch.cuda.device(self.device):
            call("mad_zone_fast_build", C.byref(s), _ptr(fast), _stream())
            torch.cuda.current_stream().synchronize()
        self.keep.append(fast)
        s.fast = fast.data_ptr()
        return s


_TABLE_CACHE = {}


def device_tables(device):
    key = (str(device),)
    if key not in _TABLE_CACHE:
        _TABLE_CACHE[key] = _DeviceTables(device)
    return _TABLE_CACHE[key]


class Space(object):

    def __init__(self):
        self.grids = []
        self.logs = []
        self.gauss = []
        self.grad4 = []
        self.grad_flags = []
        self.dims = []
        self.n_oct = 2
        self.n_input_voxels = 0
        self._gauss = []
        self._grad_done = {}

    @property
    def dims_host(self):
        return np.array([d for o in self.dims for d in o], dtype=np.int32)


def gradient_reach(radius):
    up = max(2 * radius, int(math.ceil((2 * radius - 1) * math.sqrt(3.0))) + 1)
    base = max(radius, int(math.ceil((radius - 0.5) * math.sqrt(3.0))) + 1)
    return up, base


def ensure_gradient(space, kp, radius=8):
    if all(f is None for f in space.grad_flags[:space.n_oct]) or len(kp) == 0:
        return
    key = (id(kp), int(radius))
    if key in space._grad_done:
        return
    st = _stream()
    up, base = gradient_reach(int(radius))
    f0, f1 = space.grad_flags
    if f0 is None or f1 is None:
        raise _lib.MadError("ensure_gradient: octaves must share the gradient mode")
    call("mad_gradient_mark", _ptr(kp.table), len(kp), _dptr(space.dims_host), up, base, _ptr(f0), _ptr(f1), st)
    for o, (gx, gy, gz) in enumerate(space.dims[:space.n_oct]):
        call("mad_gradient_masked", _ptr(space._gauss[o]), gx, gy, gz, _ptr(space.grad4[o]), _ptr(space.grad_flags[o]), st)
    space._grad_done[key] = kp


def full_gradient(space):
    st = _stream()
    for o, (gx, gy, gz) in enumerate(space.dims[:space.n_oct]):
        fl = space.grad_flags[o]
        if fl is None:
            continue
        fl[fl == 0] = 1
        call("mad_gradient_masked", _ptr(space._gauss[o]), gx, gy, gz, _ptr(space.grad4[o]), _ptr(fl), st)
        space.grad_flags[o] = None
    space.grad_flags = [None] * len(space.grad_flags)
    return space.grad4


def build_space(grid, map_padding=9, sig_init=2, sig_presmooth=1, exact_f64=True, keep_gauss=True, full_gradient=True,
                oct_mode="both"):
    _require_cuda()
    if isinstance(grid, np.ndarray):
        grid = torch.from_numpy(np.ascontiguousarray(grid, dtype=np.float32)).cuda()
    grid = grid.contiguous().float()
    dev = grid.device
    st = _stream()
    nx, ny, nz = grid.shape
    sp = Space()
    sp.n_input_voxels = nx * ny * nz
    if map_padding:
        bx, by, bz = nx + 2 * map_padding, ny + 2 * map_padding, nz + 2 * map_padding
        base = torch.empty((bx, by, bz), dtype=torch.float32, device=dev)
        call("mad_pad3d", _ptr(grid), nx, ny, nz, int(map_padding), _ptr(base), st)
    else:
        bx, by, bz = nx, ny, nz
        base = grid
    if oct_mode not in ("both", "up", "base"):
        raise _lib.MadError("build_space: oct_mode %r" % (oct_mode,))
    ux, uy, uz = 2 * bx - 1, 2 * by - 1, 2 * bz - 1
    if oct_mode != "base":
        up = torch.empty((ux, uy, uz), dtype=torch.float32, device=dev)
        ws_bytes = _lib.lib.mad_upsample_workspace_bytes(bx, by, bz)
        ws = torch.empty(ws_bytes, dtype=torch.uint8, device=dev)
        if sig_presmooth:
            rad = tables.gaussian_radius(sig_presmooth)
            gw = np.ascontiguousarray(tables.gaussian_weights(sig_presmooth, 0, rad))
            call("mad_upsample_presmooth", _ptr(base), bx, by, bz, _dptr(gw), rad, _ptr(up), _ptr(ws), ws_bytes, st)
        else:
            call("mad_upsample_presmooth", _ptr(base), bx, by, bz, C.c_void_p(0), 0, _ptr(up), _ptr(ws), ws_bytes, st)
        del ws
    if oct_mode == "both":
        sp.grids = [up, base]
        sp.dims = [(ux, uy, uz), (bx, by, bz)]
    else:
        sp.n_oct = 1
        sp.grids = [up] if oct_mode == "up" else [base]
        sp.dims = [(ux, uy, uz) if oct_mode == "up" else (bx, by, bz)]
    rad = tables.gaussian_radius(sig_init)
    w0 = np.ascontiguousarray(tables.gaussian_weights(sig_init, 0, rad))
    w2 = np.ascontiguousarray(tables.gaussian_weights(sig_init, 2, rad))
    scale = float(np.float32(sig_init ** 2))
    for g, (gx, gy, gz) in zip(sp.grids, sp.dims):
        ws_bytes = _lib.lib.mad_log_gauss_workspace_bytes(gx, gy, gz)
        ws = torch.empty(ws_bytes, dtype=torch.uint8, device=dev)
        lg = torch.empty((gx, gy, gz), dtype=torch.float32, device=dev)
        gs = torch.empty((gx, gy, gz), dtype=torch.float32, device=dev)
        call("mad_log_gauss", _ptr(g), gx, gy, gz, _dptr(w0), _dptr(w2), rad, C.c_float(scale), _ptr(lg), _ptr(gs),
             _ptr(ws), ws_bytes, 1 if exact_f64 else 0, st)
        del ws
        gr = torch.empty((gx, gy, gz, 4), dtype=torch.float32, device=dev)
        if full_gradient:
            call("mad_gradient", _ptr(gs), gx, gy, gz, _ptr(gr), st)
            sp.grad_flags.append(None)
        else:
            sp.grad_flags.append(torch.zeros(_lib.lib.mad_gradient_tiles(gx, gy, gz), dtype=torch.uint8, device=dev))
        sp._gauss.append(gs)
        sp.logs.append(lg)
        sp.gauss.append(gs if keep_gauss else None)
        sp.grad4.append(gr)
    if full_gradient and not keep_gauss:
        sp._gauss = []
    if sp.n_oct == 1:
        sp.dims.append((1, 1, 1))
        sp.grad4.append(torch.zeros((1, 1, 1, 4), dtype=torch.float32, device=dev))
        sp.grad_flags.append(None if full_gradient else torch.zeros(1, dtype=torch.uint8, device=dev))
    return sp


class Keypoints(object):

    def __init__(self, table, count):
        self.table = table
        self.count = int(count)
        self._host = None

    def host(self):
        if self._host is None:
            self._host = self.table[:self.count].cpu().numpy().view(KEYPOINT_DTYPE).reshape(-1)
        return self._host

    def __len__(self):
        return self.count


def keypoints_from_host(arr, device):
    arr = np.ascontiguousarray(arr, dtype=KEYPOINT_DTYPE)
    t = torch.from_numpy(arr.view(np.int32).reshape(-1, 12).copy()).to(device)
    k = Keypoints(t, len(arr))
    k._host = arr
    return k


def detect(space, border=12, threshold=5e-2, cap=None):
    _require_cuda()
    dev = space.logs[0].device
    st = _stream()
    if cap is None:
        cap = 1 << 16
    while True:
        cand = torch.empty((cap, 12), dtype=torch.int32, device=dev)
        counter = torch.zeros(1, dtype=torch.int32, device=dev)
        for o, (lg, (gx, gy, gz)) in enumerate(zip(space.logs, space.dims)):
            call("mad_detect", _ptr(lg), gx, gy, gz, o, int(border), C.c_float(threshold), _ptr(cand), cap,
                 _ptr(counter), st)
        n = _Readback.read(counter)[0]
        if n <= cap:
            break
        cap = int(n * 1.25) + 16
    out = torch.empty((max(n, 1), 12), dtype=torch.int32, device=dev)
    out_count = torch.zeros(1, dtype=torch.int32, device=dev)
    ws_bytes = _lib.lib.mad_sort_keypoints_workspace_bytes(n)
    ws = torch.empty(max(ws_bytes, 1), dtype=torch.uint8, device=dev)
    dims = space.dims_host
    call("mad_sort_keypoints", _ptr(cand), n, _dptr(dims), _ptr(out), _ptr(out_count), _ptr(ws), ws_bytes, st)
    return Keypoints(out, _Readback.read(out_count)[0])


class Oriented(object):
    def __init__(self, table, count):
        self.table = table
        self.count = int(count)
        self._host = None

    def host(self):
        if self._host is None:
            self._host = self.table[:self.count].cpu().numpy().view(ORIENTED_DTYPE).reshape(-1)
        return self._host

    def __len__(self):
        return self.count


def oriented_from_host(arr, device):
    arr = np.ascontiguousarray(arr, dtype=ORIENTED_DTYPE)
    t = torch.from_numpy(arr.view(np.int32).reshape(-1, 2).copy()).to(device)
    o = Oriented(t, len(arr))
    o._host = arr
    return o


def orient(space, kp, radius=8, lim_main=6, lim_sec=6):
    _require_cuda()
    dev = space.grad4[0].device
    st = _stream()
    tb = device_tables(dev)
    n = len(kp)
    if n == 0:
        return Oriented(torch.empty((1, 2), dtype=torch.int32, device=dev), 0)
    ensure_gradient(space, kp, radius)
    n_ori = torch.empty(n, dtype=torch.int32, device=dev)
    slots = torch.empty((n, MAX_ORI), dtype=torch.int32, device=dev)
    dims = space.dims_host
    call("mad_orient", _ptr(space.grad4[0]), _ptr(space.grad4[1]), _dptr(dims), _ptr(kp.table), n, int(radius),
         C.byref(tb.z_ori), _ptr(tb.r1), int(lim_main), int(lim_sec), _ptr(n_ori), _ptr(slots), st)
    cap = n * MAX_ORI
    out = torch.empty((cap, 2), dtype=torch.int32, device=dev)
    out_count = torch.zeros(1, dtype=torch.int32, device=dev)
    ws_bytes = _lib.lib.mad_compact_oriented_workspace_bytes(n)
    ws = torch.empty(ws_bytes, dtype=torch.uint8, device=dev)
    call("mad_compact_oriented", _ptr(n_ori), _ptr(slots), n, _ptr(out), cap, _ptr(out_count), _ptr(ws), ws_bytes, st)
    return Oriented(out, _Readback.read(out_count)[0])


def describe(space, kp, ori, radius=8):
    _require_cuda()
    dev = space.grad4[0].device
    st = _stream()
    tb = device_tables(dev)
    d = len(ori)
    dsc = torch.empty((d, DSC_LEN), dtype=torch.int16, device=dev)
    if d == 0:
        return dsc
    ensure_gradient(space, kp, radius)
    dims = space.dims_host
    call("mad_describe", _ptr(space.grad4[0]), _ptr(space.grad4[1]), _dptr(dims), _ptr(kp.table), _ptr(ori.table), d,
         int(radius), C.byref(tb.z_dsc), _ptr(tb.rf), _ptr(tb.rf_inv), tb.ori_zones, _ptr(dsc), st)
    return dsc


def describe_struct(grid, patch_size=16, map_padding=9, sig_init=2, sig_presmooth=1, exact_f64=True,
                    keep_gauss=False, full_gradient=None):
    r = (patch_size - patch_size % 2) // 2
    if full_gradient is None:
        full_gradient = bool(keep_gauss)
    sp = build_space(grid, map_padding, sig_init, sig_presmooth, exact_f64=exact_f64, keep_gauss=keep_gauss,
                     full_gradient=full_gradient)
    kp = detect(sp)
    ori = orient(sp, kp, r)
    dsc = describe(sp, kp, ori, r)
    return sp, kp, ori, dsc


class DescriptorSet(object):

    def __init__(self, dsc, need_half=False):
        _require_cuda()
        if isinstance(dsc, np.ndarray):
            dsc = torch.from_numpy(np.ascontiguousarray(dsc, dtype=np.int16)).cuda()
        self.dsc = dsc.contiguous()
        assert self.dsc.dtype == torch.int16 and self.dsc.dim() == 2 and self.dsc.shape[1] == DSC_LEN
        dev = self.dsc.device
        st = _stream()
        self.rows = self.dsc.shape[0]
        self.rows_padded = max((self.rows + 255) // 256 * 256, 256)
        self.norm2 = torch.empty(max(self.rows, 1), dtype=torch.int32, device=dev)
        self.rnorm = torch.empty(self.rows_padded, dtype=torch.float32, device=dev)
        self.u8 = torch.empty((self.rows_padded, DSC_LEN), dtype=torch.uint8, device=dev)
        mx = torch.zeros(2, dtype=torch.int32, device=dev)
        call("mad_dsc_prepare", _ptr(self.dsc), self.rows, self.rows_padded, _ptr(self.norm2), _ptr(self.rnorm),
             _ptr(self.u8), _ptr(mx), _ptr(mx[1:]), st)
        self._max_dev = mx
        self._max_entry = None
        self._max_norm2 = None
        self.half = None
        s = _lib.MadDscSet()
        s.dsc = self.dsc.data_ptr()
        s.half = 0
        s.norm2 = self.norm2.data_ptr()
        s.u8 = self.u8.data_ptr()
        s.rnorm = self.rnorm.data_ptr()
        s.rows, s.rows_padded = self.rows, self.rows_padded
        s.max_entry = -1
        s.max_norm2 = -1
        self.c = s
        if need_half:
            self.ensure_half()

    @property
    def max_entry(self):
        if self._max_entry is None:
            self._set_maxima(*self._max_dev.tolist())
        return self._max_entry

    def _set_maxima(self, max_entry, max_norm2):
        self._max_entry, self._max_norm2 = int(max_entry), int(max_norm2)
        self.c.max_entry, self.c.max_norm2 = self._max_entry, self._max_norm2

    def ensure_half(self):
        if self.half is None:
            self.half = torch.empty((self.rows_padded, DSC_LEN), dtype=torch.float16, device=self.dsc.device)
            call("mad_dsc_to_half", _ptr(self.dsc), self.rows, self.rows_padded, _ptr(self.half), _stream())
            self.c.half = self.half.data_ptr()
        return self


def _as_set(x):
    return x if isinstance(x, DescriptorSet) else DescriptorSet(x)


def _check_descriptors(hi, lo):
    if max(hi._max_entry, lo._max_entry) >= _lib.DSC_REFUSED:
        raise _lib.MadError("mad_match: not a descriptor set (a negative entry, or a squared norm >= 2^31)")


def _exact_impl(hi, lo):
    _check_descriptors(hi, lo)
    if max(hi._max_entry, lo._max_entry) <= 255:
        return 0
    if max(hi._max_entry, lo._max_entry) <= 2048 and hi._max_norm2 * lo._max_norm2 <= 1 << 48:
        return 2
    return 1


def _pick_impl(hi, lo, impl):
    verify = False
    if impl is None:
        if hi._max_entry is None or lo._max_entry is None:
            return 0, True
        impl = _exact_impl(hi, lo)
    return _pick_impl_explicit(hi, lo, impl), verify


def _pick_impl_explicit(hi, lo, impl):
    hi.max_entry, lo.max_entry
    if impl == 2:
        hi.ensure_half()
        lo.ensure_half()
    return impl


_PAIR_CAP = {}


def scores_from_dots(pair_hi, pair_lo, pair_dot, hi_norm2, lo_norm2):
    p = np.asarray(hi_norm2, dtype=np.float64)[np.asarray(pair_hi)] * np.asarray(lo_norm2, dtype=np.float64)[np.asarray(pair_lo)]
    out = np.zeros(len(p), dtype=np.float64)
    nz = p > 0.0
    out[nz] = np.asarray(pair_dot, dtype=np.float64)[nz] / np.sqrt(p[nz])
    return out


def pair_hi_from_counts(counts):
    counts = np.asarray(counts)
    return np.repeat(np.arange(len(counts), dtype=np.int32), counts)


def match_threshold(hi, lo, cc=0.6, impl=None, want="score"):
    hi, lo = _as_set(hi), _as_set(lo)
    dev = hi.dsc.device
    st = _stream()
    m = hi.rows
    if m == 0 or lo.rows == 0:
        e = torch.empty(0, dtype=torch.int32, device=dev)
        return e, e.clone(), torch.empty(0, dtype=torch.float64, device=dev)
    impl, verify = _pick_impl(hi, lo, impl)
    if impl == 0:
        return _match_threshold_onepass(hi, lo, cc, dev, st, verify, want)
    if want != "score":
        raise _lib.MadError("match_threshold: want='dot' is a format of the uint8 kernel (impl 0)")
    n_seg = int(_lib.lib.mad_match_segments(m, lo.rows, impl))
    seg_count = torch.empty(m * n_seg, dtype=torch.int32, device=dev)
    call("mad_match_count", C.byref(hi.c), C.byref(lo.c), C.c_double(cc), n_seg, _ptr(seg_count), impl, st)
    seg_off = torch.empty(m * n_seg, dtype=torch.int64, device=dev)
    total = torch.zeros(1, dtype=torch.int64, device=dev)
    ws_bytes = _lib.lib.mad_exclusive_scan_workspace_bytes(m * n_seg)
    ws = torch.empty(ws_bytes, dtype=torch.uint8, device=dev)
    call("mad_exclusive_scan_i32_to_i64", _ptr(seg_count), m * n_seg, _ptr(seg_off), _ptr(total), _ptr(ws), ws_bytes, st)
    p = int(total.item())
    pair_hi = torch.empty(max(p, 1), dtype=torch.int32, device=dev)
    pair_lo = torch.empty(max(p, 1), dtype=torch.int32, device=dev)
    score = torch.empty(max(p, 1), dtype=torch.float64, device=dev)
    call("mad_match_fill", C.byref(hi.c), C.byref(lo.c), C.c_double(cc), n_seg, _ptr(seg_off), _ptr(pair_hi), _ptr(pair_lo),
         _ptr(score), impl, st)
    return pair_hi[:p], pair_lo[:p], score[:p]


def _read_counts(count, hi, lo):
    vals = _Readback.read(count, hi._max_dev, lo._max_dev)
    hi._set_maxima(vals[1], vals[2])
    lo._set_maxima(vals[3], vals[4])
    return int(vals[0])


def _match_threshold_onepass(hi, lo, cc, dev, st, verify=False, want="score"):
    key = (hi.rows, lo.rows)
    cap = _PAIR_CAP.get(key, max(1 << 20, 16 * (hi.rows + lo.rows)))
    while True:
        cand_key = torch.empty(cap, dtype=torch.int64, device=dev)
        cand_dot = torch.empty(cap, dtype=torch.int32, device=dev)
        count = torch.empty(1, dtype=torch.int64, device=dev)
        call("mad_match_pairs", C.byref(hi.c), C.byref(lo.c), C.c_double(cc), _ptr(cand_key), _ptr(cand_dot),
             C.c_uint64(cap), _ptr(count), st)
        p = _read_counts(count, hi, lo)
        if p >= (1 << 62):
            raise _lib.MadError("mad_match_pairs: the kernel's internal hand-off timed out (pair list incomplete)")
        if verify and _exact_impl(hi, lo) != 0:
            if want != "score":
                raise _lib.MadError("match_threshold: entries above 255 need the fp16 or SIMT kernel, which have no want='dot' form")
            return match_threshold(hi, lo, cc)
        if p <= cap:
            break
        cap = p + p // 8 + 1024
    _PAIR_CAP[key] = max(cap, p + p // 4)
    pair_hi = torch.empty(max(p, 1), dtype=torch.int32, device=dev)
    pair_lo = torch.empty(max(p, 1), dtype=torch.int32, device=dev)
    score = torch.empty(max(p, 1), dtype=torch.float64 if want == "score" else torch.int32, device=dev)
    if p:
        ws_bytes = _lib.lib.mad_match_pairs_finish_workspace_bytes(p)
        ws = torch.empty(ws_bytes, dtype=torch.uint8, device=dev)
        if want == "score":
            call("mad_match_pairs_finish", _ptr(cand_key), _ptr(cand_dot), p, hi.rows, lo.rows, _ptr(hi.norm2), _ptr(lo.norm2),
                 _ptr(pair_hi), _ptr(pair_lo), _ptr(score), _ptr(ws), ws_bytes, st)
        else:
            call("mad_match_pairs_finish_dot", _ptr(cand_key), _ptr(cand_dot), p, hi.rows, lo.rows, _ptr(pair_hi), _ptr(pair_lo),
                 _ptr(score), _ptr(ws), ws_bytes, st)
    return pair_hi[:p], pair_lo[:p], score[:p]


HOST_COPY_CTAS = int(os.environ.get("MAD_HOST_COPY_CTAS", "8"))


class HostStage(object):

    def __init__(self):
        self.bufs = {}
        self.copy_stream = None
        self.keep = []

    def fetch(self, name, t, overlap=False):
        n = t.numel() * t.element_size()
        buf = self.bufs.get(name)
        if buf is None or buf.numel() < n:
            if buf is not None:
                self.keep.append(buf)
            buf = torch.empty(max(n * 5 // 4, 256), dtype=torch.uint8).pin_memory()
            self.bufs[name] = buf
        view = buf[:n].view(t.dtype).view(t.shape)
        if not n:
            return view
        if overlap:
            if self.copy_stream is None:
                self.copy_stream = torch.cuda.Stream()
            self.copy_stream.wait_stream(torch.cuda.current_stream())
            t = t.contiguous()
            if t.data_ptr() % 16 == 0:
                call("mad_copy_to_host", _ptr(t), C.c_void_p(buf.data_ptr()), n, HOST_COPY_CTAS, C.c_void_p(self.copy_stream.cuda_stream))
            else:
                with torch.cuda.stream(self.copy_stream):
                    view.copy_(t, non_blocking=True)
            t.record_stream(self.copy_stream)
            self.keep.append(t)
        else:
            view.copy_(t, non_blocking=True)
        return view

    def sync(self):
        torch.cuda.current_stream().synchronize()
        if self.copy_stream is not None:
            self.copy_stream.synchronize()
        self.keep = []
        self.marks = []

    def mark(self):
        evs = [torch.cuda.Event()]
        evs[0].record(torch.cuda.current_stream())
        if self.copy_stream is not None:
            evs.append(torch.cuda.Event())
            evs[1].record(self.copy_stream)
        self.marks = evs

    def wait(self):
        for ev in getattr(self, "marks", []):
            ev.synchronize()
        self.marks = []
        self.keep = []


class MapStream(object):

    def __init__(self, hi=None, cc=0.6, exact_f64=True, match_impl=None, patch_size=16, depth=2, download=True, compact=False):
        _require_cuda()
        self.compact = bool(compact)
        self.download = download
        self.hi = _as_set(hi) if hi is not None else None
        self.cc, self.exact, self.impl, self.patch = cc, exact_f64, match_impl, patch_size
        self.up_stream = torch.cuda.Stream()
        self.stages = [HostStage() for _ in range(max(2, depth))]
        self.n = 0
        self.gbuf = [None] * max(2, depth)
        self.gfree = [None] * max(2, depth)
        self.n_up = 0

    def upload(self, grid):
        if isinstance(grid, np.ndarray):
            grid = torch.from_numpy(np.ascontiguousarray(grid, dtype=np.float32))
        if self.n_up - self.n >= len(self.gbuf):
            raise _lib.MadError("MapStream.upload: %d uploads are waiting for submit(); the %d upload buffers are all in use"
                                % (self.n_up - self.n, len(self.gbuf)))
        k = self.n_up % len(self.gbuf)
        self.n_up += 1
        dev = torch.device("cuda", torch.cuda.current_device())
        if self.gbuf[k] is None or self.gbuf[k].shape != grid.shape:
            self.gbuf[k] = torch.empty(tuple(grid.shape), dtype=torch.float32, device=dev)
        if self.gfree[k] is not None:
            self.up_stream.wait_event(self.gfree[k])
        with torch.cuda.stream(self.up_stream):
            self.gbuf[k].copy_(grid, non_blocking=True)
            ev = torch.cuda.Event()
            ev.record(self.up_stream)
        return self.gbuf[k], ev, k

    def submit(self, uploaded):
        g, ev, k = uploaded
        cur = torch.cuda.current_stream()
        cur.wait_event(ev)
        stage = self.stages[self.n % len(self.stages)]
        self.n += 1
        stage.wait()
        sp, kp, ori, dsc = describe_struct(g, patch_size=self.patch, exact_f64=self.exact)
        if k is not None:
            self.gfree[k] = torch.cuda.Event()
            self.gfree[k].record(cur)
        get = (lambda name, t: stage.fetch(name, t, overlap=True)) if self.download else (lambda name, t: t)
        out = {"kp": get("kp", kp.table[:len(kp)]), "ori": get("ori", ori.table[:len(ori)])}
        lo = DescriptorSet(dsc) if (self.hi is not None or self.compact) else None
        if self.compact:
            out.update(dsc_u8=get("dsc8", lo.u8[:lo.rows]), lo_norm2=get("n2", lo.norm2[:lo.rows]))
        else:
            out["dsc"] = get("dsc", dsc)
        if self.hi is not None:
            if self.compact:
                ph, pl, dot = match_threshold(self.hi, lo, self.cc, impl=self.impl, want="dot")
                cnt = torch.zeros(self.hi.rows, dtype=torch.int32, device=ph.device)
                if ph.numel():
                    cnt.scatter_add_(0, ph.long(), torch.ones_like(ph))
                out.update(pair_hi_counts=get("pc", cnt), pair_lo=get("pl", pl), pair_dot=get("pd", dot))
            else:
                ph, pl, sc = match_threshold(self.hi, lo, self.cc, impl=self.impl)
                out.update(pair_hi=get("ph", ph), pair_lo=get("pl", pl), score=get("sc", sc))
        stage.mark()
        return stage, out

    def result(self, ticket):
        stage, out = ticket
        stage.wait()
        return out


class MapBatch(object):

    def __init__(self, streams=4, patch_size=16, exact_f64=True, compact=False):
        _require_cuda()
        from concurrent.futures import ThreadPoolExecutor
        self.compact = bool(compact)
        self.nw = max(1, int(streams))
        self.patch, self.exact = patch_size, exact_f64
        self.device = torch.cuda.current_device()
        self.streams = [torch.cuda.Stream() for _ in range(self.nw)]
        self.stages = [HostStage() for _ in range(self.nw)]
        self.up = [None] * self.nw
        self.pool = ThreadPoolExecutor(self.nw)
        self.last_d2h_bytes = 0
        device_tables(torch.device("cuda", self.device))

    def _work(self, w, grids, download):
        torch.cuda.set_device(self.device)
        out = []
        with torch.cuda.stream(self.streams[w]):
            for j in range(w, len(grids), self.nw):
                g = grids[j]
                if isinstance(g, np.ndarray):
                    g = torch.from_numpy(np.ascontiguousarray(g, dtype=np.float32))
                if not g.is_cuda:
                    if self.up[w] is None or self.up[w].shape != g.shape:
                        self.up[w] = torch.empty(tuple(g.shape), dtype=torch.float32, device="cuda")
                    self.up[w].copy_(g, non_blocking=True)
                    g = self.up[w]
                sp, kp, ori, dsc = describe_struct(g, patch_size=self.patch, exact_f64=self.exact)
                r = {"n_kp": len(kp), "n_dsc": len(ori)}
                if download:
                    st = self.stages[w]
                    r.update(kp=st.fetch("kp%d" % j, kp.table[:len(kp)]), ori=st.fetch("ori%d" % j, ori.table[:len(ori)]))
                    if self.compact:
                        ds = DescriptorSet(dsc)
                        r["_max"] = ds._max_dev[:1]
                        r["dsc_u8"] = st.fetch("dsc8_%d" % j, ds.u8[:ds.rows])
                        r["_dsc_dev"] = dsc
                    else:
                        r["dsc"] = st.fetch("dsc%d" % j, dsc)
                else:
                    r.update(dsc=dsc, kp=kp.table[:len(kp)], ori=ori.table[:len(ori)])
                out.append((j, r))
            self.streams[w].synchronize()
            for _, r in out:
                if "_max" in r:
                    if int(r.pop("_max").item()) > 255:
                        del r["dsc_u8"]
                        r["dsc"] = r["_dsc_dev"].cpu()
                    del r["_dsc_dev"]
        return out

    def run(self, grids, download=True):
        main = torch.cuda.current_stream()
        for s_ in self.streams:
            s_.wait_stream(main)
        parts = [f.result() for f in [self.pool.submit(self._work, w, grids, download) for w in range(self.nw)]]
        for s_ in self.streams:
            main.wait_stream(s_)
        res = [r for _, r in sorted((x for p in parts for x in p), key=lambda x: x[0])]
        if download:
            self.last_d2h_bytes = int(sum(r[k].numel() * r[k].element_size() for r in res for k in ("dsc", "dsc_u8", "kp", "ori") if k in r))
        return res


def concat_sets(sets):
    offs = np.cumsum([0] + [s.rows for s in sets]).astype(np.int64)
    return DescriptorSet(torch.cat([s.dsc for s in sets], 0)), offs


def match_topk(hi, lo, k=8, lo_index_base=0, impl=None):
    hi, lo = _as_set(hi), _as_set(lo)
    dev = hi.dsc.device
    st = _stream()
    impl, verify = _pick_impl(hi, lo, impl)
    idx = torch.empty((hi.rows, k), dtype=torch.int32, device=dev)
    score = torch.empty((hi.rows, k), dtype=torch.float64, device=dev)
    ws_bytes = _lib.lib.mad_match_topk_workspace_bytes(hi.rows, lo.rows, int(k), impl)
    ws = torch.empty(ws_bytes, dtype=torch.uint8, device=dev)
    call("mad_match_topk", C.byref(hi.c), C.byref(lo.c), int(k), int(lo_index_base), _ptr(idx), _ptr(score), _ptr(ws),
         ws_bytes, impl, st)
    if verify:
        _read_counts(torch.zeros(1, dtype=torch.int64, device=dev), hi, lo)
        if _exact_impl(hi, lo) != 0:
            return match_topk(hi, lo, k, lo_index_base)
    return idx, score


def topk_merge(idx_g, score_g):
    g, m, k = idx_g.shape
    dev = idx_g.device
    idx = torch.empty((m, k), dtype=torch.int32, device=dev)
    score = torch.empty((m, k), dtype=torch.float64, device=dev)
    call("mad_topk_merge", _ptr(idx_g.contiguous()), _ptr(score_g.contiguous()), g, m, k, _ptr(idx), _ptr(score), _stream())
    return idx, score


class FeatureTable(object):

    def __init__(self, dsc, index, oct_scale, main_bin, sec_bin, subv_map_coords):
        _require_cuda()
        self.set = dsc if isinstance(dsc, DescriptorSet) else DescriptorSet(dsc)
        dev = self.set.dsc.device
        meta = np.stack([np.asarray(index), np.asarray(oct_scale), np.asarray(main_bin), np.asarray(sec_bin)], 1)
        self.meta_host = np.ascontiguousarray(meta, dtype=np.int32)
        self.subv_host = np.ascontiguousarray(subv_map_coords, dtype=np.float64).reshape(-1, 3)
        assert len(self.meta_host) == self.set.rows == len(self.subv_host)
        self.meta = torch.from_numpy(self.meta_host).to(dev)
        self.subv = torch.from_numpy(self.subv_host).to(dev)

    @classmethod
    def from_features(cls, df_list):
        dsc = np.array([df.lin_ar_subeqsp for df in df_list], dtype=np.int16).reshape(-1, DSC_LEN)
        return cls(dsc, [df.index for df in df_list], [df.oct_scale for df in df_list], [df.main_bin for df in df_list],
                   [df.sec_bin for df in df_list], np.array([df.subv_map_coords for df in df_list], dtype=np.float64))


class AnchorCloud(object):

    def __init__(self, subv, used, cell):
        dev = subv.device
        st = _stream()
        d = int(subv.shape[0])
        self.cell = float(cell)
        self._buf = torch.empty((max(d, 1), 3), dtype=torch.float64, device=dev)
        self.org_dev = torch.empty(3, dtype=torch.float64, device=dev)
        self.info = torch.empty(8, dtype=torch.int64, device=dev)
        ws_bytes = _lib.lib.mad_anchor_cloud_workspace_bytes(d)
        ws = torch.empty(ws_bytes, dtype=torch.uint8, device=dev)
        call("mad_anchor_cloud", _ptr(subv), _ptr(used), d, C.c_double(self.cell), _ptr(self._buf), _ptr(self.org_dev),
             _ptr(self.info), _ptr(ws), ws_bytes, st)
        self.n = None

    def take_info(self, vals):
        n, bad = int(vals[0]), int(vals[1])
        if bad:
            raise _lib.MadError("anchor cloud: %d used feature(s) with a non-finite coordinate" % bad)
        self.n = n
        self.dims64 = np.array(vals[2:5], dtype=np.int64)
        self.org = np.array(vals[5:8], dtype=np.int64).view(np.float64)
        self.dims = self.dims64.astype(np.int32)
        self.cloud = self._buf[:n]
        return self

    def build_grid(self):
        dev = self._buf.device
        ncell = int(np.prod([int(v) for v in self.dims64], dtype=object))
        fits = ncell < (1 << 31)
        self.sorted = torch.empty((max(self.n, 1), 3), dtype=torch.float64, device=dev)
        self.cell_start = torch.empty(ncell + 1 if fits else 1, dtype=torch.int32, device=dev)
        self.near_bits = torch.zeros((ncell + 31) // 32 if fits else 1, dtype=torch.int32, device=dev)
        ws_bytes = _lib.lib.mad_cloud_grid_workspace_bytes(self.n)
        ws = torch.empty(ws_bytes, dtype=torch.uint8, device=dev)
        call("mad_cloud_grid", _ptr(self.cloud), self.n, _ptr(self.org_dev), _dptr(self.dims64), C.c_double(self.cell),
             _ptr(self.sorted), _ptr(self.cell_start) if fits else None, _ptr(self.near_bits) if fits else None, _ptr(ws),
             ws_bytes, _stream())
        self.sorted = self.sorted[:self.n]
        return self

    def host(self):
        return self.cloud.cpu().numpy()


def read_clouds(*clouds):
    vals = _Readback.read(*[c.info for c in clouds])
    return [c.take_info(vals[8 * i:8 * i + 8]) for i, c in enumerate(clouds)]


def anchor_cloud(subv, used, cell):
    c, = read_clouds(AnchorCloud(subv.contiguous(), used.contiguous(), cell))
    return c.build_grid()


class DscMatch(object):

    def __init__(self, lo, hi, anchor_dist_thresh=4, cc_threshold=0.65, impl=None, pairs=None):
        self.lo, self.hi = lo, hi
        self.dist = float(anchor_dist_thresh)
        dev = hi.set.dsc.device
        if pairs is None:
            pairs = match_threshold(hi.set, lo.set, cc_threshold, impl=impl)
        self.ph, self.pl, self.sc = pairs
        self.p = int(self.ph.numel())
        self.hi_cloud = self.lo_cloud = None
        if self.p == 0:
            return
        st = _stream()
        used_hi = torch.zeros(hi.set.rows, dtype=torch.uint8, device=dev)
        used_lo = torch.zeros(lo.set.rows, dtype=torch.uint8, device=dev)
        call("mad_mark_used", _ptr(self.ph), self.p, _ptr(used_hi), st)
        call("mad_mark_used", _ptr(self.pl), self.p, _ptr(used_lo), st)
        self.hi_cloud, self.lo_cloud = read_clouds(AnchorCloud(hi.subv, used_hi, self.dist),
                                                   AnchorCloud(lo.subv, used_lo, self.dist))
        self.lo_cloud.build_grid()
        self.tb = device_tables(dev)

    def _common(self):
        return (_ptr(self.hi.subv), _ptr(self.lo.subv), _ptr(self.hi.meta), _ptr(self.lo.meta), _ptr(self.tb.rf),
                _ptr(self.tb.rf_inv), self.tb.ori_zones)

    def _grid(self):
        g = self.lo_cloud
        return (_ptr(self.hi_cloud.cloud), self.hi_cloud.n, _ptr(g.sorted), _ptr(g.cell_start), _ptr(g.near_bits), _dptr(g.org),
                _dptr(g.dims), C.c_double(self.dist))

    def counts(self, p0, p1):
        out = torch.empty(max(p1 - p0, 1), dtype=torch.int32, device=self.ph.device)
        if p1 > p0:
            call("mad_repeat_counts", _ptr(self.ph), _ptr(self.pl), int(p0), int(p1), *self._common(), *self._grid(), _ptr(out),
                 _stream())
        return out[:p1 - p0]

    def rows(self, counts):
        if counts.numel() != self.p or counts.dtype != torch.int32 or counts.device != self.ph.device:
            raise _lib.MadError("DscMatch.rows: needs int32 counts of all %d pairs on %s, got %s [%d] on %s"
                                % (self.p, self.ph.device, counts.dtype, counts.numel(), counts.device))
        res = torch.empty((self.p, 23), dtype=torch.float64, device=self.ph.device)
        call("mad_repeat_rows", _ptr(self.ph), _ptr(self.pl), _ptr(self.sc), self.p, *self._common(), _ptr(counts.contiguous()),
             self.hi_cloud.n, _ptr(res), _stream())
        return res

    def table(self):
        res = torch.empty((self.p, 23), dtype=torch.float64, device=self.ph.device)
        call("mad_repeatability", _ptr(self.ph), _ptr(self.pl), _ptr(self.sc), self.p, *self._common(), *self._grid(), _ptr(res),
             _stream())
        return res

    def result(self, table):
        if self.p == 0:
            return table, np.zeros((0, 3)), np.zeros((0, 3))
        return table, self.lo_cloud.host(), self.hi_cloud.host()

    def empty(self):
        return torch.empty((0, 23), dtype=torch.float64, device=self.ph.device)


def match_dsc(lo, hi, anchor_dist_thresh=4, cc_threshold=0.65, impl=None):
    m = DscMatch(lo, hi, anchor_dist_thresh, cc_threshold, impl)
    return m.result(m.table() if m.p else m.empty())


def match_dsc_lists(lo_dsc_list, hi_dsc_list, anchor_dist_thresh=4, cc_threshold=0.65):
    res, lo_cloud, hi_cloud = match_dsc(FeatureTable.from_features(lo_dsc_list), FeatureTable.from_features(hi_dsc_list),
                                        anchor_dist_thresh, cc_threshold)
    return list(res.cpu().numpy()), lo_cloud, hi_cloud
```

Before: 2.240 billion.

## Replace radix sort of match pairs with per-row run counts and merge placement

The pair-matching kernel now records, for each candidate, its rank within a per-row, per-segment, per-group run, plus per-row run counts. The finish step computes row offsets with a block scan and places each pair directly, merging two sorted column groups by binary search. This replaces the cub radix sort over 64-bit keys. The cost is extra rank and count bookkeeping (ballots, match_any) in the hot epilogue, an extra rank buffer, and several small kernels. Debug flags that zero the mask and dot values were also added.

```diff
diff --git a/include/mad_b200.h b/include/mad_b200.h
--- a/include/mad_b200.h
+++ b/include/mad_b200.h
@@ -134,15 +134,17 @@
 int mad_exclusive_scan_i32_to_i64(const int32_t* in, int n, int64_t* out, int64_t* total,
                                   void* workspace, size_t workspace_bytes, void* stream);
 
+int mad_match_pairs_runs(const MadDscSet* hi, const MadDscSet* lo, int* n_seg, int* seg_cols);
 int mad_match_pairs(const MadDscSet* hi, const MadDscSet* lo, double cc, uint64_t* cand_key, int32_t* cand_dot,
-                    uint64_t cap, uint64_t* count, void* stream);
-size_t mad_match_pairs_finish_workspace_bytes(long long n);
-int mad_match_pairs_finish(const uint64_t* cand_key, const int32_t* cand_dot, long long n, int hi_rows, int lo_rows,
-                           const int32_t* hi_n2, const int32_t* lo_n2, int32_t* pair_hi, int32_t* pair_lo,
-                           double* pair_score, void* workspace, size_t workspace_bytes, void* stream);
-int mad_match_pairs_finish_dot(const uint64_t* cand_key, const int32_t* cand_dot, long long n, int hi_rows, int lo_rows,
-                               int32_t* pair_hi, int32_t* pair_lo, int32_t* pair_dot, void* workspace, size_t workspace_bytes,
-                               void* stream);
+                    int32_t* cand_rank, int32_t* run_count, uint64_t cap, uint64_t* count, void* stream);
+size_t mad_match_pairs_finish_workspace_bytes(long long n, int hi_rows);
+int mad_match_pairs_finish(const uint64_t* cand_key, const int32_t* cand_dot, const int32_t* cand_rank, const int32_t* run_count,
+                           int n_seg, int seg_cols, long long n, int hi_rows, const int32_t* hi_n2, const int32_t* lo_n2,
+                           int32_t* pair_hi, int32_t* pair_lo, double* pair_score, void* workspace, size_t workspace_bytes,
+                           void* stream);
+int mad_match_pairs_finish_dot(const uint64_t* cand_key, const int32_t* cand_dot, const int32_t* cand_rank,
+                               const int32_t* run_count, int n_seg, int seg_cols, long long n, int hi_rows, int32_t* pair_hi,
+                               int32_t* pair_lo, int32_t* pair_dot, void* workspace, size_t workspace_bytes, void* stream);
 
 size_t mad_match_topk_workspace_bytes(int M, int N, int k, int impl);
 int mad_match_topk(const MadDscSet* hi, const MadDscSet* lo, int k, int lo_index_base,
diff --git a/mad_b200/_lib.py b/mad_b200/_lib.py
--- a/mad_b200/_lib.py
+++ b/mad_b200/_lib.py
@@ -79,10 +79,11 @@
     "mad_compact_oriented": (_I, [_P, _P, _I, _P, _I, _P, _P, _SZ, _P]),
     "mad_describe": (_I, [_P, _P, _P, _P, _P, _I, _I, C.POINTER(MadZoneTable), _P, _P, _I, _P, _P]),
     "mad_dsc_prepare": (_I, [_P, _I, _I, _P, _P, _P, _P, _P, _P]),
-    "mad_match_pairs": (_I, [C.POINTER(MadDscSet), C.POINTER(MadDscSet), C.c_double, _P, _P, C.c_uint64, _P, _P]),
-    "mad_match_pairs_finish_workspace_bytes": (_SZ, [C.c_longlong]),
-    "mad_match_pairs_finish": (_I, [_P, _P, C.c_longlong, _I, _I, _P, _P, _P, _P, _P, _P, _SZ, _P]),
-    "mad_match_pairs_finish_dot": (_I, [_P, _P, C.c_longlong, _I, _I, _P, _P, _P, _P, _SZ, _P]),
+    "mad_match_pairs_runs": (_I, [C.POINTER(MadDscSet), C.POINTER(MadDscSet), _P, _P]),
+    "mad_match_pairs": (_I, [C.POINTER(MadDscSet), C.POINTER(MadDscSet), C.c_double, _P, _P, _P, _P, C.c_uint64, _P, _P]),
+    "mad_match_pairs_finish_workspace_bytes": (_SZ, [C.c_longlong, _I]),
+    "mad_match_pairs_finish": (_I, [_P, _P, _P, _P, _I, _I, C.c_longlong, _I, _P, _P, _P, _P, _P, _P, _SZ, _P]),
+    "mad_match_pairs_finish_dot": (_I, [_P, _P, _P, _P, _I, _I, C.c_longlong, _I, _P, _P, _P, _P, _SZ, _P]),
     "mad_dsc_norms": (_I, [_P, _I, _P, _P]),
     "mad_dsc_to_half": (_I, [_P, _I, _I, _P, _P]),
     "mad_match_segments": (_I, [_I, _I, _I]),
diff --git a/mad_b200/csrc/match_common.cuh b/mad_b200/csrc/match_common.cuh
--- a/mad_b200/csrc/match_common.cuh
+++ b/mad_b200/csrc/match_common.cuh
@@ -124,9 +124,11 @@
 
 int mad_match_u8_segments(int M, int N);
 int mad_match_u8_segments_topk(int M, int N);
+void mad_match_u8_pairs_runs(int M, int N, int N_pad, int* n_seg, int* seg_cols);
 int mad_match_u8_pairs(const void* hi_u8, int M, int M_pad, const void* lo_u8, int N, int N_pad, const int32_t* hi_n2,
                        const int32_t* lo_n2, const float* lo_rnorm, double cc, unsigned long long* cand_key,
-                       int32_t* cand_dot, unsigned long long cap, unsigned long long* count, cudaStream_t st);
+                       int32_t* cand_dot, int32_t* cand_rank, int32_t* run_count, unsigned long long cap,
+                       unsigned long long* count, cudaStream_t st);
 int mad_match_u8_topk(const void* hi_u8, int M, int M_pad, const void* lo_u8, int N, int N_pad, const int32_t* hi_n2,
                       const int32_t* lo_n2, const float* lo_rnorm, int S, int k, int lo_index_base, int32_t* topk_idx,
                       double* topk_score, cudaStream_t st);
diff --git a/mad_b200/csrc/match_prep.cu b/mad_b200/csrc/match_prep.cu
--- a/mad_b200/csrc/match_prep.cu
+++ b/mad_b200/csrc/match_prep.cu
@@ -1,4 +1,4 @@
-#include <cub/cub.cuh>
+#include <cub/block/block_scan.cuh>
 
 #include "common.cuh"
 #include "match_common.cuh"
@@ -56,48 +56,102 @@
     }
 }
 
-__global__ void pairs_finish_kernel(const unsigned long long* __restrict__ key, const int32_t* __restrict__ dot,
-                                    long long n, unsigned long long lo_rows, const int32_t* __restrict__ hi_n2,
-                                    const int32_t* __restrict__ lo_n2,
-                                    int32_t* __restrict__ pair_hi, int32_t* __restrict__ pair_lo,
-                                    double* __restrict__ score) {
+constexpr int ROWS_BLK = 256;
+
+__global__ void __launch_bounds__(ROWS_BLK)
+pairs_rows_kernel(const int32_t* __restrict__ run_count, int n_runs, int M, long long* __restrict__ row_off,
+                  long long* __restrict__ blk_off) {
+    using Scan = cub::BlockScan<long long, ROWS_BLK>;
+    __shared__ typename Scan::TempStorage tmp;
+    const int row = blockIdx.x * ROWS_BLK + threadIdx.x;
+    long long t = 0;
+    if (row < M)
+        for (int r = 0; r < n_runs; ++r) t += run_count[(long long)r * M + row];
+    long long ex, agg;
+    Scan(tmp).ExclusiveSum(t, ex, agg);
+    if (row < M) row_off[row] = ex;
+    if (threadIdx.x == 0) blk_off[blockIdx.x] = agg;
+}
+
+__global__ void __launch_bounds__(ROWS_BLK) pairs_scan_kernel(long long* __restrict__ blk_off, int nb) {
+    using Scan = cub::BlockScan<long long, ROWS_BLK>;
+    __shared__ typename Scan::TempStorage tmp;
+    long long carry = 0;
+    for (int base = 0; base < nb; base += ROWS_BLK) {
+        const int i = base + threadIdx.x;
+        long long ex, agg;
+        Scan(tmp).ExclusiveSum(i < nb ? blk_off[i] : 0ll, ex, agg);
+        if (i < nb) blk_off[i] = carry + ex;
+        carry += agg;
+        __syncthreads();
+    }
+}
+
+struct PairPlace {
+    int row, col, g;
+    long long seg_start;
+    long long c0, c1;
+};
+
+__device__ __forceinline__ PairPlace pair_place(unsigned long long key, const int32_t* __restrict__ run_count, int M, int seg_cols,
+                                                const long long* __restrict__ row_off, const long long* __restrict__ blk_off) {
+    PairPlace q;
+    q.row = (int)(key >> 32);
+    q.col = (int)(unsigned)key;
+    const int s = q.col / seg_cols;
+    q.g = ((q.col - s * seg_cols) >> 7) & 1;
+    long long b = row_off[q.row] + blk_off[q.row / ROWS_BLK];
+    for (int r = 0; r < 2 * s; ++r) b += __ldg(run_count + (long long)r * M + q.row);
+    q.seg_start = b;
+    q.c0 = __ldg(run_count + (long long)(2 * s) * M + q.row);
+    q.c1 = __ldg(run_count + (long long)(2 * s + 1) * M + q.row);
+    return q;
+}
+
+__global__ void pairs_runs_kernel(const unsigned long long* __restrict__ key, const int32_t* __restrict__ rank, long long n,
+                                  const int32_t* __restrict__ run_count, int M, int seg_cols, const long long* __restrict__ row_off,
+                                  const long long* __restrict__ blk_off, int32_t* __restrict__ run_col) {
     const long long i = blockIdx.x * (long long)blockDim.x + threadIdx.x;
     if (i >= n) return;
-    const unsigned long long k = key[i];
-    const int row = (int)(k / lo_rows), col = (int)(k % lo_rows);
-    pair_hi[i] = row;
-    pair_lo[i] = col;
-    score[i] = mad_score(dot[i], (double)__ldg(hi_n2 + row), (double)__ldg(lo_n2 + col));
-}
-
-__global__ void pairs_finish_dot_kernel(const unsigned long long* __restrict__ key, const int32_t* __restrict__ dot, long long n,
-                                        unsigned long long lo_rows, int32_t* __restrict__ pair_hi, int32_t* __restrict__ pair_lo,
-                                        int32_t* __restrict__ pair_dot) {
+    const PairPlace q = pair_place(key[i], run_count, M, seg_cols, row_off, blk_off);
+    run_col[q.seg_start + (q.g ? q.c0 : 0) + rank[i]] = q.col;
+}
+
+__global__ void pairs_finish_kernel(const unsigned long long* __restrict__ key, const int32_t* __restrict__ dot,
+                                    const int32_t* __restrict__ rank, long long n, const int32_t* __restrict__ run_count, int M,
+                                    int seg_cols, const long long* __restrict__ row_off, const long long* __restrict__ blk_off,
+                                    const int32_t* __restrict__ run_col, const int32_t* __restrict__ hi_n2,
+                                    const int32_t* __restrict__ lo_n2, int32_t* __restrict__ pair_hi, int32_t* __restrict__ pair_lo,
+                                    double* __restrict__ score, int32_t* __restrict__ pair_dot) {
     const long long i = blockIdx.x * (long long)blockDim.x + threadIdx.x;
     if (i >= n) return;
-    const unsigned long long k = key[i];
-    pair_hi[i] = (int)(k / lo_rows);
-    pair_lo[i] = (int)(k % lo_rows);
-    pair_dot[i] = dot[i];
+    const PairPlace q = pair_place(key[i], run_count, M, seg_cols, row_off, blk_off);
+    const int32_t* other = run_col + q.seg_start + (q.g ? 0 : q.c0);
+    long long lo = 0, hi = q.g ? q.c0 : q.c1;
+    while (lo < hi) {
+        const long long mid = (lo + hi) >> 1;
+        if (other[mid] < q.col) lo = mid + 1; else hi = mid;
+    }
+    const long long o = q.seg_start + rank[i] + lo;
+    pair_hi[o] = q.row;
+    pair_lo[o] = q.col;
+    if (hi_n2) score[o] = mad_score(dot[i], (double)__ldg(hi_n2 + q.row), (double)__ldg(lo_n2 + q.col));
+    else pair_dot[o] = dot[i];
 }
 
 __global__ void zero_u64_kernel(unsigned long long* p) { *p = 0ull; }
 
 struct FinishLayout {
-    size_t key_off, dot_off, cub_off, cub_bytes, total;
+    size_t col_off, row_off, blk_off, total;
 };
 
-FinishLayout finish_layout(long long n) {
+FinishLayout finish_layout(long long n, int hi_rows) {
     FinishLayout L;
-    const size_t nn = (size_t)(n > 0 ? n : 1);
-    L.key_off = 0;
-    L.dot_off = mad_align_up(nn * sizeof(unsigned long long), 256);
-    L.cub_off = L.dot_off + mad_align_up(nn * sizeof(int32_t), 256);
-    size_t b = 0;
-    cub::DeviceRadixSort::SortPairs(nullptr, b, (const unsigned long long*)nullptr, (unsigned long long*)nullptr,
-                                    (const int32_t*)nullptr, (int32_t*)nullptr, (int)nn, 0, 64);
-    L.cub_bytes = mad_align_up(b, 256);
-    L.total = L.cub_off + L.cub_bytes;
+    const size_t nn = (size_t)(n > 0 ? n : 1), m = (size_t)(hi_rows > 0 ? hi_rows : 1);
+    L.col_off = 0;
+    L.row_off = mad_align_up(nn * sizeof(int32_t), 256);
+    L.blk_off = L.row_off + mad_align_up(m * sizeof(long long), 256);
+    L.total = L.blk_off + mad_align_up((size_t)mad_ceil_div((long long)m, ROWS_BLK) * sizeof(long long), 256);
     return L;
 }
 
@@ -116,8 +170,14 @@
     return MAD_OK;
 }
 
+extern "C" int mad_match_pairs_runs(const MadDscSet* hi, const MadDscSet* lo, int* n_seg, int* seg_cols) {
+    MAD_CHECK_ARG(hi && lo && n_seg && seg_cols && hi->rows >= 0 && lo->rows >= 0);
+    mad_match_u8_pairs_runs(hi->rows, lo->rows, lo->rows_padded, n_seg, seg_cols);
+    return MAD_OK;
+}
+
 extern "C" int mad_match_pairs(const MadDscSet* hi, const MadDscSet* lo, double cc, uint64_t* cand_key, int32_t* cand_dot,
-                               uint64_t cap, uint64_t* count, void* stream) {
+                               int32_t* cand_rank, int32_t* run_count, uint64_t cap, uint64_t* count, void* stream) {
     MAD_CHECK_ARG(hi && lo && count && hi->rows >= 0 && lo->rows >= 0);
     cudaStream_t st = (cudaStream_t)stream;
     {
@@ -126,7 +186,7 @@
         MAD_LAUNCH_OK();
     }
     if (hi->rows == 0 || lo->rows == 0) return MAD_OK;
-    MAD_CHECK_ARG(hi->u8 && lo->u8 && hi->norm2 && lo->norm2 && lo->rnorm && cand_key && cand_dot);
+    MAD_CHECK_ARG(hi->u8 && lo->u8 && hi->norm2 && lo->norm2 && lo->rnorm && cand_key && cand_dot && cand_rank && run_count);
     MAD_CHECK_ARG(hi->rows_padded >= hi->rows && hi->rows_padded % 128 == 0);
     MAD_CHECK_ARG(lo->rows_padded >= lo->rows && lo->rows_padded % 128 == 0);
     int rc = mad_check_descriptor_sets(hi, lo, "mad_match_pairs");
@@ -138,61 +198,66 @@
         return MAD_ERR_ARG;
     }
     return mad_match_u8_pairs(hi->u8, hi->rows, hi->rows_padded, lo->u8, lo->rows, lo->rows_padded, hi->norm2, lo->norm2,
-                              lo->rnorm, cc, reinterpret_cast<unsigned long long*>(cand_key), cand_dot,
+                              lo->rnorm, cc, reinterpret_cast<unsigned long long*>(cand_key), cand_dot, cand_rank, run_count,
                               (unsigned long long)cap, reinterpret_cast<unsigned long long*>(count), st);
 }
 
-extern "C" size_t mad_match_pairs_finish_workspace_bytes(long long n) { return finish_layout(n).total; }
-
-static int pairs_finish_impl(const uint64_t* cand_key, const int32_t* cand_dot, long long n, int hi_rows, int lo_rows,
-                             const int32_t* hi_n2, const int32_t* lo_n2, int32_t* pair_hi, int32_t* pair_lo, double* pair_score,
-                             int32_t* pair_dot, void* workspace, size_t workspace_bytes, void* stream);
-
-extern "C" int mad_match_pairs_finish(const uint64_t* cand_key, const int32_t* cand_dot, long long n, int hi_rows,
-                                      int lo_rows, const int32_t* hi_n2, const int32_t* lo_n2, int32_t* pair_hi, int32_t* pair_lo,
-                                      double* pair_score, void* workspace, size_t workspace_bytes, void* stream) {
+extern "C" size_t mad_match_pairs_finish_workspace_bytes(long long n, int hi_rows) { return finish_layout(n, hi_rows).total; }
+
+static int pairs_finish_impl(const uint64_t* cand_key, const int32_t* cand_dot, const int32_t* cand_rank, const int32_t* run_count,
+                             int n_seg, int seg_cols, long long n, int hi_rows, const int32_t* hi_n2, const int32_t* lo_n2,
+                             int32_t* pair_hi, int32_t* pair_lo, double* pair_score, int32_t* pair_dot, void* workspace,
+                             size_t workspace_bytes, void* stream) {
     MAD_CHECK_ARG(n >= 0 && n < (1LL << 31));
     if (n == 0) return MAD_OK;
-    MAD_CHECK_ARG(hi_n2 && lo_n2 && pair_score);
-    return pairs_finish_impl(cand_key, cand_dot, n, hi_rows, lo_rows, hi_n2, lo_n2, pair_hi, pair_lo, pair_score, nullptr, workspace,
-                             workspace_bytes, stream);
-}
-
-extern "C" int mad_match_pairs_finish_dot(const uint64_t* cand_key, const int32_t* cand_dot, long long n, int hi_rows, int lo_rows,
-                                          int32_t* pair_hi, int32_t* pair_lo, int32_t* pair_dot, void* workspace,
-                                          size_t workspace_bytes, void* stream) {
-    MAD_CHECK_ARG(n >= 0 && n < (1LL << 31));
-    if (n == 0) return MAD_OK;
-    MAD_CHECK_ARG(pair_dot);
-    return pairs_finish_impl(cand_key, cand_dot, n, hi_rows, lo_rows, nullptr, nullptr, pair_hi, pair_lo, nullptr, pair_dot, workspace,
-                             workspace_bytes, stream);
-}
-
-static int pairs_finish_impl(const uint64_t* cand_key, const int32_t* cand_dot, long long n, int hi_rows, int lo_rows,
-                             const int32_t* hi_n2, const int32_t* lo_n2, int32_t* pair_hi, int32_t* pair_lo, double* pair_score,
-                             int32_t* pair_dot, void* workspace, size_t workspace_bytes, void* stream) {
-    MAD_CHECK_ARG(cand_key && cand_dot && pair_hi && pair_lo && workspace && hi_rows > 0 && lo_rows > 0);
-    const FinishLayout L = finish_layout(n);
+    MAD_CHECK_ARG(cand_key && cand_dot && cand_rank && run_count && pair_hi && pair_lo && workspace && hi_rows > 0);
+    MAD_CHECK_ARG(n_seg >= 1 && seg_cols > 0 && seg_cols % 128 == 0);
+    const FinishLayout L = finish_layout(n, hi_rows);
     MAD_CHECK_ARG(workspace_bytes >= L.total);
     cudaStream_t st = (cudaStream_t)stream;
     char* ws = reinterpret_cast<char*>(workspace);
-    unsigned long long* key_sorted = reinterpret_cast<unsigned long long*>(ws + L.key_off);
-    int32_t* dot_sorted = reinterpret_cast<int32_t*>(ws + L.dot_off);
-    int key_bits = 1;
-    while (key_bits < 64 && (1ULL << key_bits) < (unsigned long long)hi_rows * (unsigned long long)lo_rows) ++key_bits;
-    size_t b = L.cub_bytes;
-    {
-        MAD_PROF("cub_radix_sort_pairs", st);
-        MAD_CUDA(cub::DeviceRadixSort::SortPairs(ws + L.cub_off, b, reinterpret_cast<const unsigned long long*>(cand_key),
-                                                 key_sorted, cand_dot, dot_sorted, (int)n, 0, key_bits, st));
+    int32_t* run_col = reinterpret_cast<int32_t*>(ws + L.col_off);
+    long long* row_off = reinterpret_cast<long long*>(ws + L.row_off);
+    long long* blk_off = reinterpret_cast<long long*>(ws + L.blk_off);
+    const int nb = (int)mad_ceil_div(hi_rows, ROWS_BLK);
+    const unsigned long long* key = reinterpret_cast<const unsigned long long*>(cand_key);
+    const unsigned grid = (unsigned)mad_ceil_div(n, 256);
+    {
+        MAD_PROF("pairs_rows_kernel", st);
+        pairs_rows_kernel<<<nb, ROWS_BLK, 0, st>>>(run_count, 2 * n_seg, hi_rows, row_off, blk_off);
+        MAD_LAUNCH_OK();
+    }
+    {
+        MAD_PROF("pairs_scan_kernel", st);
+        pairs_scan_kernel<<<1, ROWS_BLK, 0, st>>>(blk_off, nb);
+        MAD_LAUNCH_OK();
+    }
+    {
+        MAD_PROF("pairs_runs_kernel", st);
+        pairs_runs_kernel<<<grid, 256, 0, st>>>(key, cand_rank, n, run_count, hi_rows, seg_cols, row_off, blk_off, run_col);
+        MAD_LAUNCH_OK();
     }
     MAD_PROF("pairs_finish_kernel", st);
-    if (pair_dot)
-        pairs_finish_dot_kernel<<<(unsigned)mad_ceil_div(n, 256), 256, 0, st>>>(key_sorted, dot_sorted, n, (unsigned long long)lo_rows, pair_hi,
-                                                                               pair_lo, pair_dot);
-    else
-        pairs_finish_kernel<<<(unsigned)mad_ceil_div(n, 256), 256, 0, st>>>(key_sorted, dot_sorted, n, (unsigned long long)lo_rows, hi_n2, lo_n2,
-                                                                           pair_hi, pair_lo, pair_score);
+    pairs_finish_kernel<<<grid, 256, 0, st>>>(key, cand_dot, cand_rank, n, run_count, hi_rows, seg_cols, row_off, blk_off, run_col,
+                                              hi_n2, lo_n2, pair_hi, pair_lo, pair_score, pair_dot);
     MAD_LAUNCH_OK();
     return MAD_OK;
 }
+
+extern "C" int mad_match_pairs_finish(const uint64_t* cand_key, const int32_t* cand_dot, const int32_t* cand_rank,
+                                      const int32_t* run_count, int n_seg, int seg_cols, long long n, int hi_rows,
+                                      const int32_t* hi_n2, const int32_t* lo_n2, int32_t* pair_hi, int32_t* pair_lo,
+                                      double* pair_score, void* workspace, size_t workspace_bytes, void* stream) {
+    MAD_CHECK_ARG(n == 0 || (hi_n2 && lo_n2 && pair_score));
+    return pairs_finish_impl(cand_key, cand_dot, cand_rank, run_count, n_seg, seg_cols, n, hi_rows, hi_n2, lo_n2, pair_hi, pair_lo,
+                             pair_score, nullptr, workspace, workspace_bytes, stream);
+}
+
+extern "C" int mad_match_pairs_finish_dot(const uint64_t* cand_key, const int32_t* cand_dot, const int32_t* cand_rank,
+                                          const int32_t* run_count, int n_seg, int seg_cols, long long n, int hi_rows,
+                                          int32_t* pair_hi, int32_t* pair_lo, int32_t* pair_dot, void* workspace,
+                                          size_t workspace_bytes, void* stream) {
+    MAD_CHECK_ARG(n == 0 || pair_dot);
+    return pairs_finish_impl(cand_key, cand_dot, cand_rank, run_count, n_seg, seg_cols, n, hi_rows, nullptr, nullptr, pair_hi, pair_lo,
+                             nullptr, pair_dot, workspace, workspace_bytes, stream);
+}
diff --git a/mad_b200/csrc/match_u8.cu b/mad_b200/csrc/match_u8.cu
--- a/mad_b200/csrc/match_u8.cu
+++ b/mad_b200/csrc/match_u8.cu
@@ -145,6 +145,8 @@
     double cc;
     unsigned long long* cand_key;
     int32_t* cand_dot;
+    int32_t* cand_rank;
+    int32_t* run_count;
     unsigned long long cap;
     unsigned long long* count;
     int k, lo_index_base;
@@ -280,62 +282,88 @@
         }
     } else if (warp >= 2 && warp < 4 && MODE == MODE_PAIRS) {
         constexpr int HALF = STG / 2;
-        const int e0 = (warp - 2) * 4;
+        const int grp = warp - 2;
+        const int e0 = grp * 4;
         const double cc2 = a.cc * a.cc;
+        const unsigned lt = (1u << lane) - 1u;
         int hi_n2_reg[4];
-#pragma unroll
-        for (int qq = 0; qq < 4; ++qq) hi_n2_reg[qq] = (m0 + qq * 32 + lane < a.M) ? __ldg(a.hi_n2 + m0 + qq * 32 + lane) : 0;
+        int run_n[4];
+#pragma unroll
+        for (int qq = 0; qq < 4; ++qq) {
+            hi_n2_reg[qq] = (m0 + qq * 32 + lane < a.M) ? __ldg(a.hi_n2 + m0 + qq * 32 + lane) : 0;
+            run_n[qq] = 0;
+        }
+        unsigned next_half = 0;
         for (long long spins = 0; spins < (1LL << 27); ++spins) {
             int done = 0;
             for (int e = e0; e < e0 + 4; ++e) done += mad_ld_acquire_cta(&s_done[e]);
             bool any = false;
-            for (int e = e0; e < e0 + 4; ++e) {
-                for (int h = 0; h < 2; ++h) {
-                    const int n = mad_ld_acquire_cta(&s_half[2 * e + h]);
-                    if (n <= 0) continue;
-                    any = true;
-                    const unsigned long long* hk = stg_key + e * STG + h * HALF;
-                    const int* hd = stg_dot + e * STG + h * HALF;
-                    unsigned long long ent[2];
-                    int dot[2];
-                    bool ok[2];
-#pragma unroll
-                    for (int k = 0; k < 2; ++k) {
-                        const int i = lane + 32 * k;
-                        ent[k] = (i < n) ? hk[i] : 0ull;
-                        dot[k] = (i < n) ? hd[i] : 0;
-                    }
-                    __syncwarp();
-                    if (lane == 0) mad_st_release_cta(&s_half[2 * e + h], 0);
-                    int total = 0, pos[2];
-                    const int qe = e & 3;
-                    const int n2_q = qe == 0 ? hi_n2_reg[0] : (qe == 1 ? hi_n2_reg[1] : (qe == 2 ? hi_n2_reg[2] : hi_n2_reg[3]));
-#pragma unroll
-                    for (int k = 0; k < 2; ++k) {
-                        ok[k] = false;
-                        const unsigned low = (unsigned)ent[k];
-                        const double n2r = (double)__shfl_sync(0xFFFFFFFFu, n2_q, (int)(low & 31u));
-                        if (lane + 32 * k < n) {
-                            const int row = m0 + qe * 32 + (int)(low & 31u);
-                            const double n2c = (double)(unsigned)(ent[k] >> 32);
-                            const double p = n2r * n2c, lhs = (double)dot[k] * (double)dot[k], rhs = cc2 * p;
-                            if (p > 0.0 && a.cc > 0.0 && lhs > rhs * (1.0 + 1e-13)) ok[k] = true;
-                            else if (p > 0.0 && a.cc > 0.0 && lhs < rhs * (1.0 - 1e-13)) ok[k] = false;
-                            else ok[k] = mad_score(dot[k], n2r, n2c) > a.cc;
-                            ent[k] = (unsigned long long)row * (unsigned long long)a.N + (unsigned long long)(low >> 5);
+            for (int qe = 0; qe < 4; ++qe) {
+                const int e = e0 + qe;
+                const int h = (next_half >> qe) & 1;
+                const int n = mad_ld_acquire_cta(&s_half[2 * e + h]);
+                if (n <= 0) continue;
+                any = true;
+                next_half ^= 1u << qe;
+                const unsigned long long* hk = stg_key + e * STG + h * HALF;
+                const int* hd = stg_dot + e * STG + h * HALF;
+                unsigned long long ent[2];
+                int dot[2], rank[2];
+                bool ok[2];
+#pragma unroll
+                for (int k = 0; k < 2; ++k) {
+                    const int i = lane + 32 * k;
+                    ent[k] = (i < n) ? hk[i] : 0ull;
+                    dot[k] = (i < n) ? hd[i] : 0;
+                }
+                __syncwarp();
+                if (lane == 0) mad_st_release_cta(&s_half[2 * e + h], 0);
+                if (a.dbg & 256) continue;
+                int total = 0, pos[2];
+                const int n2_q = qe == 0 ? hi_n2_reg[0] : (qe == 1 ? hi_n2_reg[1] : (qe == 2 ? hi_n2_reg[2] : hi_n2_reg[3]));
+                int cnt = qe == 0 ? run_n[0] : (qe == 1 ? run_n[1] : (qe == 2 ? run_n[2] : run_n[3]));
+#pragma unroll
+                for (int k = 0; k < 2; ++k) {
+                    ok[k] = false;
+                    const unsigned low = (unsigned)ent[k];
+                    const int r = (int)(low & 31u);
+                    const double n2r = (double)__shfl_sync(0xFFFFFFFFu, n2_q, r);
+                    if (lane + 32 * k < n) {
+                        const int row = m0 + qe * 32 + r;
+                        const double n2c = (double)(unsigned)(ent[k] >> 32);
+                        const double p = n2r * n2c, lhs = (double)dot[k] * (double)dot[k], rhs = cc2 * p;
+                        if (p > 0.0 && a.cc > 0.0 && lhs > rhs * (1.0 + 1e-13)) ok[k] = true;
+                        else if (p > 0.0 && a.cc > 0.0 && lhs < rhs * (1.0 - 1e-13)) ok[k] = false;
+                        else ok[k] = mad_score(dot[k], n2r, n2c) > a.cc;
+                        ent[k] = ((unsigned long long)row << 32) | (unsigned long long)(low >> 5);
+                    }
+                    const unsigned m = __ballot_sync(0xFFFFFFFFu, ok[k]);
+                    pos[k] = total + __popc(m & lt);
+                    total += __popc(m);
+                    const unsigned peers = __match_any_sync(0xFFFFFFFFu, ok[k] ? r : 32 + lane) & m;
+                    rank[k] = __shfl_sync(0xFFFFFFFFu, cnt, r) + __popc(peers & lt);
+                    unsigned mine = m;
+#pragma unroll
+                    for (int b = 0; b < 5; ++b) {
+                        const unsigned bb = __ballot_sync(0xFFFFFFFFu, (r >> b) & 1);
+                        mine &= ((lane >> b) & 1) ? bb : ~bb;
+                    }
+                    cnt += __popc(mine);
+                }
+#pragma unroll
+                for (int qq = 0; qq < 4; ++qq)
+                    if (qq == qe) run_n[qq] = cnt;
+                if (total > 0) {
+                    unsigned long long gb = 0;
+                    if (lane == 0) gb = atomicAdd(a.count, (unsigned long long)total);
+                    gb = __shfl_sync(0xFFFFFFFFu, gb, 0);
+#pragma unroll
+                    for (int k = 0; k < 2; ++k)
+                        if (ok[k] && gb + pos[k] < a.cap) {
+                            a.cand_key[gb + pos[k]] = ent[k];
+                            a.cand_dot[gb + pos[k]] = dot[k];
+                            a.cand_rank[gb + pos[k]] = rank[k];
                         }
-                        const unsigned m = __ballot_sync(0xFFFFFFFFu, ok[k]);
-                        pos[k] = total + __popc(m & ((1u << lane) - 1u));
-                        total += __popc(m);
-                    }
-                    if (total > 0) {
-                        unsigned long long gb = 0;
-                        if (lane == 0) gb = atomicAdd(a.count, (unsigned long long)total);
-                        gb = __shfl_sync(0xFFFFFFFFu, gb, 0);
-#pragma unroll
-                        for (int k = 0; k < 2; ++k)
-                            if (ok[k] && gb + pos[k] < a.cap) { a.cand_key[gb + pos[k]] = ent[k]; a.cand_dot[gb + pos[k]] = dot[k]; }
-                    }
                 }
             }
             if (!any) {
@@ -344,6 +372,9 @@
             }
             if (spins == (1LL << 27) - 1 && lane == 0) atomicExch(a.count, MAD_MATCH_TIMEOUT_COUNT);
         }
+#pragma unroll
+        for (int qq = 0; qq < 4; ++qq)
+            if (m0 + qq * 32 + lane < a.M) a.run_count[(long long)(seg * 2 + grp) * a.M + m0 + qq * 32 + lane] = run_n[qq];
     } else if ((warp == 2 || warp == 3 || warp >= 4 + EPI_WARPS) && MODE == MODE_TOP8) {
         const int dq = warp < 4 ? warp - 2 : warp - (4 + EPI_WARPS) + 2;
         float ts[8];
@@ -613,6 +644,7 @@
                 } else {
                     const int left = a.N - (n0 + c0);
                     if (left < 32) mask &= (left <= 0) ? 0u : ((1u << left) - 1u);
+                    if (a.dbg & 128) mask = 0u;
                     const unsigned lt = (1u << lane) - 1u;
                     for (;;) {
                         const unsigned b = __ballot_sync(0xFFFFFFFFu, mask != 0u);
@@ -625,7 +657,7 @@
                             const int p = cur * HALF + stg_n + __popc(b & lt);
                             my_key[p] = ((unsigned long long)(unsigned)__float_as_int(rbt[c0 + j + 128]) << 32) |
                                         (unsigned long long)(((unsigned)(n0 + c0 + j) << 5) | (unsigned)lane);
-                            my_dot[p] = (int)mad_select32(v, j);
+                            my_dot[p] = (a.dbg & 512) ? 0 : (int)mad_select32(v, j);
                         }
                         stg_n += nb;
                     }
@@ -796,9 +828,16 @@
     return MAD_OK;
 }
 
+void mad_match_u8_pairs_runs(int M, int N, int N_pad, int* n_seg, int* seg_cols) {
+    const int ncta = pick_ncta(M, N_pad);
+    *n_seg = mad_match_u8_segments(M, N);
+    *seg_cols = (int)mad_ceil_div(mad_ceil_div(N, BN * ncta), *n_seg) * BN * ncta;
+}
+
 int mad_match_u8_pairs(const void* hi_u8, int M, int M_pad, const void* lo_u8, int N, int N_pad, const int32_t* hi_n2,
                        const int32_t* lo_n2, const float* lo_rnorm, double cc, unsigned long long* cand_key,
-                       int32_t* cand_dot, unsigned long long cap, unsigned long long* count, cudaStream_t st) {
+                       int32_t* cand_dot, int32_t* cand_rank, int32_t* run_count, unsigned long long cap,
+                       unsigned long long* count, cudaStream_t st) {
     CUtensorMap map_hi, map_lo;
     const int ncta = pick_ncta(M, N_pad);
     int rc = launch_common(hi_u8, M_pad, lo_u8, N_pad, ncta, &map_hi, &map_lo);
@@ -806,10 +845,11 @@
     if (N_pad > (1 << 27)) { mad_set_error("mad_match_pairs: more than 2^27 lo rows"); return MAD_ERR_ARG; }
     U8Args a = {};
     a.M = M; a.N = N;
-    a.S = mad_match_u8_segments(M, N);
-    a.tiles_per_seg = (int)mad_ceil_div(mad_ceil_div(N, BN * ncta), a.S);
+    int seg_cols = 0;
+    mad_match_u8_pairs_runs(M, N, N_pad, &a.S, &seg_cols);
+    a.tiles_per_seg = seg_cols / (BN * ncta);
     a.hi_n2 = hi_n2; a.lo_n2 = lo_n2; a.lo_rnorm = lo_rnorm; a.cc = cc;
-    a.cand_key = cand_key; a.cand_dot = cand_dot; a.cap = cap; a.count = count;
+    a.cand_key = cand_key; a.cand_dot = cand_dot; a.cand_rank = cand_rank; a.run_count = run_count; a.cap = cap; a.count = count;
     a.dbg = getenv("MAD_TOPK_DBG") ? atoi(getenv("MAD_TOPK_DBG")) : 0;
     MAD_PROF("match_u8_pairs_kernel", st);
     return launch_u8<MODE_PAIRS>(ncta, M, a.S, map_hi, map_lo, a, st);
diff --git a/mad_b200/pipeline.py b/mad_b200/pipeline.py
--- a/mad_b200/pipeline.py
+++ b/mad_b200/pipeline.py
@@ -508,12 +508,16 @@
 def _match_threshold_onepass(hi, lo, cc, dev, st, verify=False, want="score"):
     key = (hi.rows, lo.rows)
     cap = _PAIR_CAP.get(key, max(1 << 20, 16 * (hi.rows + lo.rows)))
+    n_seg, seg_cols = C.c_int(), C.c_int()
+    call("mad_match_pairs_runs", C.byref(hi.c), C.byref(lo.c), C.byref(n_seg), C.byref(seg_cols))
+    run_count = torch.empty(2 * n_seg.value * hi.rows, dtype=torch.int32, device=dev)
     while True:
         cand_key = torch.empty(cap, dtype=torch.int64, device=dev)
         cand_dot = torch.empty(cap, dtype=torch.int32, device=dev)
+        cand_rank = torch.empty(cap, dtype=torch.int32, device=dev)
         count = torch.empty(1, dtype=torch.int64, device=dev)
-        call("mad_match_pairs", C.byref(hi.c), C.byref(lo.c), C.c_double(cc), _ptr(cand_key), _ptr(cand_dot),
-             C.c_uint64(cap), _ptr(count), st)
+        call("mad_match_pairs", C.byref(hi.c), C.byref(lo.c), C.c_double(cc), _ptr(cand_key), _ptr(cand_dot), _ptr(cand_rank),
+             _ptr(run_count), C.c_uint64(cap), _ptr(count), st)
         p = _read_counts(count, hi, lo)
         if p >= (1 << 62):
             raise _lib.MadError("mad_match_pairs: the kernel's internal hand-off timed out (pair list incomplete)")
@@ -529,14 +533,14 @@
     pair_lo = torch.empty(max(p, 1), dtype=torch.int32, device=dev)
     score = torch.empty(max(p, 1), dtype=torch.float64 if want == "score" else torch.int32, device=dev)
     if p:
-        ws_bytes = _lib.lib.mad_match_pairs_finish_workspace_bytes(p)
+        ws_bytes = _lib.lib.mad_match_pairs_finish_workspace_bytes(p, hi.rows)
         ws = torch.empty(ws_bytes, dtype=torch.uint8, device=dev)
+        runs = (_ptr(cand_key), _ptr(cand_dot), _ptr(cand_rank), _ptr(run_count), n_seg.value, seg_cols.value, p, hi.rows)
         if want == "score":
-            call("mad_match_pairs_finish", _ptr(cand_key), _ptr(cand_dot), p, hi.rows, lo.rows, _ptr(hi.norm2), _ptr(lo.norm2),
-                 _ptr(pair_hi), _ptr(pair_lo), _ptr(score), _ptr(ws), ws_bytes, st)
+            call("mad_match_pairs_finish", *runs, _ptr(hi.norm2), _ptr(lo.norm2), _ptr(pair_hi), _ptr(pair_lo), _ptr(score),
+                 _ptr(ws), ws_bytes, st)
         else:
-            call("mad_match_pairs_finish_dot", _ptr(cand_key), _ptr(cand_dot), p, hi.rows, lo.rows, _ptr(pair_hi), _ptr(pair_lo),
-                 _ptr(score), _ptr(ws), ws_bytes, st)
+            call("mad_match_pairs_finish_dot", *runs, _ptr(pair_hi), _ptr(pair_lo), _ptr(score), _ptr(ws), ws_bytes, st)
     return pair_hi[:p], pair_lo[:p], score[:p]
 
 
```

Measured after the change: 2.234 billion, median of 6. Within noise of the previous version (-0.3%).
